# amolahinge/739-839-federated-learning-using-grpc

Measured on AMD Instinct MI355X. Metric: rounds/sec + samples/sec/client, 2-conv CNN FedAvg at 1/2/4/8 MI355X clients, higher is better.
Workload: dtype bf16; 1 GPU; model=lenet, global_batch=128, parallelism=fedavg-dp1, per_client_batch=128, local_epochs_per_round=1, eval_per_round=True, eval_split=full-per-client, data_split=strided-iid, aggregation=none (single client), hip_graph=True

## Files before the change

### csrc/bindings.cpp

```cpp
#include <pybind11/pybind11.h>
#include <pybind11/stl.h>

#include <hip/hip_runtime.h>
#include <stdint.h>
#include <cmath>
#include <vector>

#include "kernels/common.h"
#include "kernels/lenet_layout.h"
#include "runtime/lenet_engine.h"

namespace py = pybind11;

namespace fedmi {
void launch_lenet_conv_fwd(hipStream_t, const uint8_t*, int, int, const bf16*, const float*, uint32_t, const int*, int,
                           bf16*, bf16*, int, bf16*, uint8_t*, uint8_t*, lenet::Stats*);
void launch_lenet_fc_eval(hipStream_t, const bf16*, const int*, int, const bf16*, const float*, float*, long,
                          lenet::Stats*);
bool stamps_enabled();
void read_stamps(unsigned long long*, bool);
void set_ks1_diag(int);
void launch_lenet_pack(hipStream_t, const float*, bf16*);
void launch_sgd_flat(hipStream_t, float*, const float*, float*, long, float, float, float, float, int, int);
void launch_server_opt(hipStream_t, float*, float*, float*, float*, long, long, int, float, float, float, float);
void launch_drift_grad(hipStream_t, int, float*, const float*, const float*, const float*, float*, float, long);
void launch_scaffold_finish(hipStream_t, const float*, float*, float*, long, long);
void launch_scaffold_begin(hipStream_t, float*, const float*, const float*, float*, float*, long);
int dp_partials(long);
void launch_dp(hipStream_t, float*, const float*, long, double*, double*, double, float, uint64_t, uint64_t, int);
int robust_partials(long);
void launch_robust_reduce(hipStream_t, const float*, long, int, long, int, float*, long long*, long long*);
void launch_ef_delta(hipStream_t, const float*, const float*, const float*, float*, long);
size_t topk_state_bytes();
size_t topk_overflow_offset();
void launch_topk_ef(hipStream_t, const float*, const float*, float*, long, int, void*, int*, unsigned*, int*, float*);
void launch_scatter_add_ranked(hipStream_t, float*, const int*, const float*, int, long, float, long);
void launch_quant_int8(hipStream_t, const float*, long, signed char*, float*, float*);
void launch_dequant_accum(hipStream_t, const signed char*, const float*, int, long, float*, float);
}

using namespace fedmi;

void fedmi_bind_cnn(py::module_& m);
void fedmi_bind_comm(py::module_& m);
void fedmi_bind_zoo(py::module_& m);
void fedmi_bind_io(py::module_& m);

template <typename T>
static T* P(uintptr_t p) { return reinterpret_cast<T*>(p); }
static hipStream_t S(uintptr_t s) { return reinterpret_cast<hipStream_t>(s); }

static void check_last(const char* what) { check_hip(hipGetLastError(), what); }

static LeNetBuffers buffers_from(const py::dict& d) {
  auto get = [&](const char* k) -> uintptr_t { return d.contains(k) ? d[k].cast<uintptr_t>() : 0; };
  LeNetBuffers b;
  b.train_images = P<const uint8_t>(get("train_images"));
  b.train_labels = P<const int>(get("train_labels"));
  b.n_train = d.contains("n_train") ? d["n_train"].cast<int>() : 0;
  b.params = P<float>(get("params"));
  b.mom = P<float>(get("mom"));
  b.pk = P<bf16>(get("pk"));
  b.act2 = P<bf16>(get("act2"));
  b.act2_rows = d.contains("act2_rows") ? d["act2_rows"].cast<int>() : 0;
  b.act2T = P<bf16>(get("act2T"));
  b.h1 = P<bf16>(get("h1"));
  b.dact2 = P<float>(get("dact2"));
  b.dZ1T = P<bf16>(get("dZ1T"));
  b.conv_slab = P<float>(get("conv_slab"));
  b.eval_part = P<float>(get("eval_part"));
  b.eval_part_floats = d.contains("eval_part_floats") ? d["eval_part_floats"].cast<long>() : 0;
  b.train_stats = P<lenet::Stats>(get("train_stats"));
  b.eval_stats = P<lenet::Stats>(get("eval_stats"));
  b.round_ctr = P<int>(get("round_ctr"));
  return b;
}

static void fedmi_bind(py::module_& m) {
  fedmi_bind_cnn(m);
  fedmi_bind_comm(m);
  fedmi_bind_zoo(m);
  fedmi_bind_io(m);
  m.def("stamps_enabled", &stamps_enabled);
  m.def("set_ks1_diag", &set_ks1_diag);
  m.def("read_stamps", [](bool clear) {
    const size_t n = (size_t)FEDMI_STAMP_KERNELS * FEDMI_STAMP_WGS * FEDMI_STAMP_SLOTS;
    std::vector<unsigned long long> buf(n, 0ull);
    read_stamps(buf.data(), clear);
    return py::bytes(reinterpret_cast<const char*>(buf.data()), n * sizeof(unsigned long long));
  }, py::arg("clear") = true);
  m.attr("STAMP_SHAPE") = py::make_tuple(FEDMI_STAMP_KERNELS, FEDMI_STAMP_WGS, FEDMI_STAMP_SLOTS);
  m.doc() = "fedmi native runtime: fused LeNet HIP kernels, graph executor, flat-buffer and compression kernels (gfx950)";

  m.def("lenet_layout", []() {
    using namespace lenet;
    py::dict d;
    d["P_C1W"] = P_C1W; d["P_C1B"] = P_C1B; d["P_C2W"] = P_C2W; d["P_C2B"] = P_C2B;
    d["P_F1W"] = P_F1W; d["P_F1B"] = P_F1B; d["P_F2W"] = P_F2W; d["P_F2B"] = P_F2B;
    d["P_F3W"] = P_F3W; d["P_F3B"] = P_F3B; d["P_TOTAL"] = P_TOTAL;
    d["CS"] = CS; d["FS"] = FS; d["F1W_N"] = F1W_N; d["DZ1_LD"] = DZ1_LD; d["PK_TOTAL"] = PK_TOTAL; d["F0"] = F0; d["F0P"] = F0P; d["NP1"] = NP1;
    d["MAX_TRAIN_BATCH"] = MAX_TRAIN_BATCH; d["FC_SPW"] = FC_SPW;
    d["IMG_BYTES"] = IMG_BYTES; d["STATS_BYTES"] = (int)sizeof(Stats);
    return d;
  });

  py::class_<SgdConfig>(m, "SgdConfig")
      .def(py::init<>())
      .def_readwrite("lr", &SgdConfig::lr)
      .def_readwrite("momentum", &SgdConfig::momentum)
      .def_readwrite("weight_decay", &SgdConfig::weight_decay);

  py::class_<LeNetEngine>(m, "LeNetEngine")
      .def(py::init([](const py::dict& bufs, float lr, float momentum, float wd, uint32_t seed, bool augment) {
             SgdConfig c;
             c.lr = lr; c.momentum = momentum; c.weight_decay = wd;
             return new LeNetEngine(buffers_from(bufs), c, seed, augment);
           }),
           py::arg("buffers"), py::arg("lr"), py::arg("momentum"), py::arg("weight_decay"), py::arg("seed"),
           py::arg("augment"))
      .def("set_schedule", &LeNetEngine::set_schedule)
      .def("schedule_len", &LeNetEngine::schedule_len)
      .def("step", [](LeNetEngine& e, uintptr_t st, int start, int nb, bool bump, bool reset) {
             e.step(S(st), start, nb, bump, reset);
           }, py::arg("stream"), py::arg("start"), py::arg("nb"), py::arg("bump_round") = false,
           py::arg("reset_stats") = false,
           py::call_guard<py::gil_scoped_release>())
      .def("run_epoch", [](LeNetEngine& e, uintptr_t st, bool use_graph) { e.run_epoch(S(st), use_graph); },
           py::call_guard<py::gil_scoped_release>())
      .def("eval", [](LeNetEngine& e, uintptr_t st, uintptr_t images, uintptr_t labels, int n) {
             e.eval(S(st), P<const uint8_t>(images), P<const int>(labels), n);
           }, py::arg("st"), py::arg("images"), py::arg("labels"), py::arg("n"), py::call_guard<py::gil_scoped_release>())
      .def("pack", [](LeNetEngine& e, uintptr_t st) { e.pack(S(st)); }, py::call_guard<py::gil_scoped_release>())
      .def("set_sgd", [](LeNetEngine& e, float lr, float m, float wd) {
             SgdConfig c; c.lr = lr; c.momentum = m; c.weight_decay = wd; e.set_sgd(c);
           })
      .def("graph_ready", &LeNetEngine::graph_ready);

  m.def("lenet_conv_fwd", [](uintptr_t st, uintptr_t images, int base, int nb, uintptr_t pk, uintptr_t params,
                             uint32_t seed, uintptr_t round_ctr, int augment, uintptr_t act2, uintptr_t act2T,
                             int tstride, uintptr_t pool1, uintptr_t am1, uintptr_t am2, uintptr_t zero_stats) {
    launch_lenet_conv_fwd(S(st), P<const uint8_t>(images), base, nb, P<const bf16>(pk), P<const float>(params), seed,
                          P<const int>(round_ctr), augment, P<bf16>(act2), P<bf16>(act2T), tstride, P<bf16>(pool1),
                          P<uint8_t>(am1), P<uint8_t>(am2), P<lenet::Stats>(zero_stats));
    check_last("lenet_conv_fwd");
  });
  m.def("lenet_pack", [](uintptr_t st, uintptr_t params, uintptr_t pk) {
    launch_lenet_pack(S(st), P<const float>(params), P<bf16>(pk));
    check_last("lenet_pack");
  });

  m.def("sgd_flat", [](uintptr_t st, uintptr_t p, uintptr_t g, uintptr_t buf, long n, float lr, float mo, float wd,
                       float damp, bool nesterov, bool first) {
    launch_sgd_flat(S(st), P<float>(p), P<const float>(g), P<float>(buf), n, lr, mo, wd, damp, nesterov ? 1 : 0,
                    first ? 1 : 0);
    check_last("sgd_flat");
  });
  m.def("server_opt", [](uintptr_t st, uintptr_t x, uintptr_t anchor, uintptr_t mom, uintptr_t v, long n, long n_opt,
                         int kind, float lr, float beta1, float beta2, float tau) {
    if (kind < 0 || kind > 3) throw std::invalid_argument("server_opt: kind must be 0..3");
    if (n < 0 || n_opt < 0 || n_opt > n) throw std::invalid_argument("server_opt: need 0 <= n_opt <= n");
    if (n == 0) return;
    if (!x || !anchor || !mom || (kind != 0 && !v)) throw std::invalid_argument("server_opt: null buffer");
    if ((x | anchor | mom | v) % 16) throw std::invalid_argument("server_opt: buffers must be 16-byte aligned");
    launch_server_opt(S(st), P<float>(x), P<float>(anchor), P<float>(mom), P<float>(v), n, n_opt, kind, lr, beta1,
                      beta2, tau);
    check_last("server_opt");
  }, py::arg("stream"), py::arg("x"), py::arg("anchor"), py::arg("m"), py::arg("v"), py::arg("n"), py::arg("n_opt"),
     py::arg("kind"), py::arg("lr"), py::arg("beta1"), py::arg("beta2"), py::arg("tau"));

  m.def("dp_partials", [](long k) {
    if (k < 0) throw std::invalid_argument("dp_partials: need k >= 0");
    return dp_partials(k);
  });
  m.def("dp_privatize", [](uintptr_t st, uintptr_t x, uintptr_t anchor, long n, long k, uintptr_t partial,
                           uintptr_t stats, double clip, double z, int world, uint64_t key, uint64_t draw, int stages) {
    if (n < 0 || k < 0 || k > n) throw std::invalid_argument("dp_privatize: need 0 <= k <= n");
    if (!(clip > 0.0) || !std::isfinite(clip)) throw std::invalid_argument("dp_privatize: need a finite clip norm S > 0");
    if (!(z >= 0.0) || !std::isfinite(z)) throw std::invalid_argument("dp_privatize: need a finite noise multiplier z >= 0");
    if (world < 1) throw std::invalid_argument("dp_privatize: need world >= 1");
    if (stages < 1 || stages > 7) throw std::invalid_argument("dp_privatize: stages must be in 1..7");
    if (k == 0) return;
    if (!x || !anchor || !partial || !stats) throw std::invalid_argument("dp_privatize: null buffer");
    if ((x | anchor) % 16) throw std::invalid_argument("dp_privatize: x and anchor must be 16-byte aligned");
    if ((partial | stats) % 8) throw std::invalid_argument("dp_privatize: partial and stats must be 8-byte aligned");
    const float sigma = (float)(z * clip / std::sqrt((double)world));
    launch_dp(S(st), P<float>(x), P<const float>(anchor), k, P<double>(partial), P<double>(stats), clip, sigma, key,
              draw, stages);
    check_last("dp_privatize");
  }, py::arg("stream"), py::arg("x"), py::arg("anchor"), py::arg("n"), py::arg("k"), py::arg("partial"),
     py::arg("stats"), py::arg("clip"), py::arg("z"), py::arg("world"), py::arg("key"), py::arg("draw"),
     py::arg("stages") = 7);

  m.def("robust_partials", [](long n) {
    if (n < 0) throw std::invalid_argument("robust_partials: need n >= 0");
    return robust_partials(n);
  });
  m.def("robust_reduce", [](uintptr_t st, uintptr_t rows, long ld, int W, long n, int b_eff, uintptr_t out,
                            uintptr_t partial, uintptr_t stats) {
    if (W < 2 || W > 16) throw std::invalid_argument("robust_reduce: W must be in 2..16");
    if (b_eff < 0 || b_eff > (W - 1) / 2) throw std::invalid_argument("robust_reduce: need 0 <= b_eff <= (W - 1) / 2");
    if (n < 0) throw std::invalid_argument("robust_reduce: need n >= 0");
    if (ld < n || ld % 4) throw std::invalid_argument("robust_reduce: the row stride ld must be >= n and a multiple of 4");
    if (!rows || !out || !partial || !stats) throw std::invalid_argument("robust_reduce: null buffer");
    if ((rows | out) % 16) throw std::invalid_argument("robust_reduce: rows and out must be 16-byte aligned");
    if ((partial | stats) % 8) throw std::invalid_argument("robust_reduce: partial and stats must be 8-byte aligned");
    if (n == 0) return;
    launch_robust_reduce(S(st), P<const float>(rows), ld, W, n, b_eff, P<float>(out), P<long long>(partial),
                         P<long long>(stats));
    check_last("robust_reduce");
  }, py::arg("stream"), py::arg("rows"), py::arg("ld"), py::arg("W"), py::arg("n"), py::arg("b_eff"), py::arg("out"),
     py::arg("partial"), py::arg("stats"));

  m.def("drift_grad", [](uintptr_t st, int kind, uintptr_t g, uintptr_t p, uintptr_t anchor, uintptr_t corr,
                         uintptr_t acc, float mu, long n) {
    if (kind < 0 || kind > 1) throw std::invalid_argument("drift_grad: kind must be 0 (fedprox) or 1 (scaffold)");
    if (n < 0) throw std::invalid_argument("drift_grad: need n >= 0");
    if (n == 0) return;
    if (!g || (kind == 0 ? (!p || !anchor) : (!corr || !acc))) throw std::invalid_argument("drift_grad: null buffer");
    if ((g | p | anchor | corr | acc) % 16) throw std::invalid_argument("drift_grad: buffers must be 16-byte aligned");
    launch_drift_grad(S(st), kind, P<float>(g), P<const float>(p), P<const float>(anchor), P<const float>(corr),
                      P<float>(acc), mu, n);
    check_last("drift_grad");
  }, py::arg("stream"), py::arg("kind"), py::arg("g"), py::arg("p"), py::arg("anchor"), py::arg("corr"),
     py::arg("acc"), py::arg("mu"), py::arg("n"));
  m.def("scaffold_finish", [](uintptr_t st, uintptr_t acc, uintptr_t ci, uintptr_t delta, long K, long n) {
    if (K < 1) throw std::invalid_argument("scaffold_finish: need K >= 1 (no SGD step was counted this round)");
    if (n < 0) throw std::invalid_argument("scaffold_finish: need n >= 0");
    if (n == 0) return;
    if (!acc || !ci || !delta) throw std::invalid_argument("scaffold_finish: null buffer");
    if ((acc | ci | delta) % 16) throw std::invalid_argument("scaffold_finish: buffers must be 16-byte aligned");
    launch_scaffold_finish(S(st), P<const float>(acc), P<float>(ci), P<float>(delta), K, n);
    check_last("scaffold_finish");
  }, py::arg("stream"), py::arg("acc"), py::arg("ci"), py::arg("delta"), py::arg("K"), py::arg("n"));
  m.def("scaffold_begin", [](uintptr_t st, uintptr_t c, uintptr_t dmean, uintptr_t ci, uintptr_t corr, uintptr_t acc,
                             long n) {
    if (n < 0) throw std::invalid_argument("scaffold_begin: need n >= 0");
    if (n == 0) return;
    if (!c || !dmean || !ci || !corr || !acc) throw std::invalid_argument("scaffold_begin: null buffer");
    if ((c | dmean | ci | corr | acc) % 16) throw std::invalid_argument("scaffold_begin: buffers must be 16-byte aligned");
    launch_scaffold_begin(S(st), P<float>(c), P<const float>(dmean), P<const float>(ci), P<float>(corr),
                          P<float>(acc), n);
    check_last("scaffold_begin");
  }, py::arg("stream"), py::arg("c"), py::arg("dmean"), py::arg("ci"), py::arg("corr"), py::arg("acc"), py::arg("n"));

  m.def("topk_state_bytes", &topk_state_bytes);
  m.def("topk_overflow_offset", &topk_overflow_offset);
  m.def("topk_ef", [](uintptr_t st, uintptr_t x, uintptr_t g, uintptr_t residual, long n, int k, uintptr_t state,
                      uintptr_t cidx, uintptr_t ckey, uintptr_t idx, uintptr_t val) {
    if (k <= 0 || k > n) throw std::invalid_argument("topk_ef: need 0 < k <= n");
    if (n >= (1L << 30)) throw std::invalid_argument("topk_ef: n must be < 2^30 (int32 indices, 2n scratch)");
    if (!x || !g || !residual || !state || !cidx || !ckey || !idx || !val) throw std::invalid_argument("topk_ef: null buffer");
    launch_topk_ef(S(st), P<const float>(x), P<const float>(g), P<float>(residual), n, k, P<void>(state), P<int>(cidx),
                   P<unsigned>(ckey), P<int>(idx), P<float>(val));
    check_last("topk_ef");
  }, py::arg("stream"), py::arg("x"), py::arg("g"), py::arg("residual"), py::arg("n"), py::arg("k"), py::arg("state"),
     py::arg("cidx"), py::arg("ckey"), py::arg("idx"), py::arg("val"));
  m.def("ef_delta", [](uintptr_t st, uintptr_t local, uintptr_t global, uintptr_t residual, uintptr_t d, long n) {
    if (n < 0) throw std::invalid_argument("ef_delta: need n >= 0");
    if (n == 0) return;
    if (!local || !global || !d) throw std::invalid_argument("ef_delta: null buffer (only residual may be 0)");
    launch_ef_delta(S(st), P<const float>(local), P<const float>(global), P<const float>(residual), P<float>(d), n);
    check_last("ef_delta");
  });
  m.def("scatter_add_ranked", [](uintptr_t st, uintptr_t out, uintptr_t idx, uintptr_t val, int R, long m_, float scale,
                                 long n) {
    if (R <= 0) throw std::invalid_argument("scatter_add_ranked: R must be > 0");
    if (m_ < 0 || n < 0) throw std::invalid_argument("scatter_add_ranked: need m >= 0 and n >= 0");
    if (m_ == 0 || n == 0) return;
    if (!out || !idx || !val) throw std::invalid_argument("scatter_add_ranked: null buffer");
    launch_scatter_add_ranked(S(st), P<float>(out), P<const int>(idx), P<const float>(val), R, m_, scale, n);
    check_last("scatter_add_ranked");
  });
  m.def("quant_int8", [](uintptr_t st, uintptr_t d, long n, uintptr_t q, uintptr_t scales, uintptr_t residual) {
    if (n < 0) throw std::invalid_argument("quant_int8: need n >= 0");
    if (n == 0) return;
    if (!d || !q || !scales) throw std::invalid_argument("quant_int8: null buffer (only residual may be 0)");
    launch_quant_int8(S(st), P<const float>(d), n, P<signed char>(q), P<float>(scales), P<float>(residual));
    check_last("quant_int8");
  });
  m.def("dequant_accum", [](uintptr_t st, uintptr_t q, uintptr_t scales, int R, long n, uintptr_t out, float scale) {
    if (R <= 0) throw std::invalid_argument("dequant_accum: R must be > 0");
    if (n < 0) throw std::invalid_argument("dequant_accum: need n >= 0");
    if (n == 0) return;
    if (!q || !scales || !out) throw std::invalid_argument("dequant_accum: null buffer");
    launch_dequant_accum(S(st), P<const signed char>(q), P<const float>(scales), R, n, P<float>(out), scale);
    check_last("dequant_accum");
  });
}

#ifndef FEDMI_MODULE
#define FEDMI_MODULE _fedmi_native
#endif
PYBIND11_MODULE(FEDMI_MODULE, m) { fedmi_bind(m); }
```

### csrc/kernels/lenet_kernels.hip

```cpp
#include <stdexcept>

#include "common.h"
#include "lenet_layout.h"

using namespace lenet;

#ifdef FEDMI_STAMPS
__device__ unsigned long long fedmi_stamps[FEDMI_STAMP_KERNELS][FEDMI_STAMP_WGS][FEDMI_STAMP_SLOTS];
__device__ int fedmi_ks1_diag;
#endif

namespace {

constexpr int NT_FWD = 512;
constexpr int NW_FWD = NT_FWD / 64;
constexpr int NT_CONV = 1024;
constexpr int NW_CONV = NT_CONV / 64;
constexpr int NT_FC = 512;

__constant__ float kMean[3] = {0.4914f, 0.4822f, 0.4465f};
__constant__ float kInvStd[3] = {1.f / 0.2023f, 1.f / 0.1994f, 1.f / 0.2010f};

FEDMI_DEV bf16x8 ld8(const bf16* p) { return *reinterpret_cast<const bf16x8*>(p); }

FEDMI_DEV bf16x8 ld8_b64x2(const bf16* p) {
  typedef __bf16 bf16x4 __attribute__((ext_vector_type(4)));
  const bf16x4 lo = *reinterpret_cast<const bf16x4*>(p);
  const bf16x4 hi = *reinterpret_cast<const bf16x4*>(p + 4);
  bf16x8 r;
#pragma unroll
  for (int j = 0; j < 4; ++j) { r[j] = lo[j]; r[j + 4] = hi[j]; }
  return r;
}

struct Aug { int i0, j0, flip; };
FEDMI_DEV Aug aug_params(int augment, uint32_t seed, const int* round_ctr, int gidx) {
  Aug a{4, 4, 0};
  if (augment) {
    const uint32_t h = hash3(seed, (uint32_t)round_ctr[0], (uint32_t)gidx);
    a.i0 = (int)(h % 9u);
    a.j0 = (int)((h >> 8) % 9u);
    a.flip = (int)((h >> 16) & 1u);
  }
  return a;
}

FEDMI_DEV float aug_pixel(const uint8_t* raw, const Aug& a, int c, int y, int x) {
  const int sy = y + a.i0 - 4;
  const int sx = (a.flip ? 31 - x : x) + a.j0 - 4;
  float v = 0.f;
  if (sy >= 0 && sy < IMG && sx >= 0 && sx < IMG) v = (float)raw[c * 1024 + sy * 32 + sx] * (1.f / 255.f);
  return (v - kMean[c]) * kInvStd[c];
}

FEDMI_DEV void load_raw(const uint8_t* __restrict__ img, uint8_t* raw) {
  if ((int)threadIdx.x < IMG_BYTES / 16)
    reinterpret_cast<uint4*>(raw)[threadIdx.x] = reinterpret_cast<const uint4*>(img)[threadIdx.x];
}

template <int NT>
FEDMI_DEV void zero_lds(void* p, int bytes) {
  uint4* q = reinterpret_cast<uint4*>(p);
  const uint4 z = make_uint4(0, 0, 0, 0);
  for (int e = threadIdx.x; e < bytes / 16; e += NT) q[e] = z;
}

}

__global__ __launch_bounds__(NT_FWD, 6) void lenet_conv_fwd(
    const uint8_t* __restrict__ images, int sample_base, int nb,
    const bf16* __restrict__ pk, const float* __restrict__ params,
    uint32_t seed, const int* __restrict__ round_ctr, int augment,
    bf16* __restrict__ act2,
    bf16* __restrict__ act2T,
    int tstride,
    bf16* __restrict__ pool1_out,
    uint8_t* __restrict__ am1_out,
    uint8_t* __restrict__ am2_out,
    Stats* __restrict__ zero_stats)
{
  constexpr int XCL = 36 * 40 * 4, P1CL = 14 * 14 * 8;
  constexpr int O_X = 3072, O_C1 = O_X + XCL * 2, O_P1 = O_C1 + NPOS1 * 8 * 4, O_C2 = O_P1 + P1CL * 2,
                O_END = O_C2 + C2 * NPOS2 * 4;
  __shared__ __attribute__((aligned(16))) unsigned char smem[O_END];
  uint8_t* raw = smem;
  bf16* xcl = reinterpret_cast<bf16*>(smem + O_X);
  float* c1 = reinterpret_cast<float*>(smem + O_C1);
  bf16* p1cl = reinterpret_cast<bf16*>(smem + O_P1);
  float* c2 = reinterpret_cast<float*>(smem + O_C2);

  const int s = blockIdx.x;
  if (s >= nb) return;
  [[maybe_unused]] const int stamp_wg = s;
  const int gidx = sample_base + s;
  const int tid = threadIdx.x, lane = lane_id(), wave = wave_id();
  const int kq = (lane >> 4) * 8, n16 = lane & 15, rq = (lane >> 4) * 4;
  if (zero_stats != nullptr && s == 0 && tid == 0) *zero_stats = Stats{0.f, 0, 0, 0};
  FEDMI_STAMP(0, 0);

  bf16x8 wr1[4], wr2[7];
  load_raw(images + (size_t)gidx * IMG_BYTES, raw);
  zero_lds<NT_FWD>(xcl, XCL * 2);
#pragma unroll
  for (int ks = 0; ks < 4; ++ks) wr1[ks] = ld8(pk + PK_W1C + n16 * K1C + ks * 32 + kq);
#pragma unroll
  for (int ks = 0; ks < 7; ++ks) wr2[ks] = ld8(pk + PK_W2C + n16 * K2C + ks * 32 + kq);
  int go1[4], go2[7];
#pragma unroll
  for (int ks = 0; ks < 4; ++ks) {
    const int g = ks * 4 + (lane >> 4);
    go1[ks] = g < 15 ? ((g / 3) * 40 + 2 * (g % 3)) * 4 : 0;
  }
#pragma unroll
  for (int ks = 0; ks < 7; ++ks) {
    const int g = ks * 4 + (lane >> 4);
    go2[ks] = g < 25 ? ((g / 5) * P1 + (g % 5)) * 8 : 0;
  }
  const float bias1 = n16 < C1 ? params[P_C1B + n16] : 0.f;
  const float bias2 = params[P_C2B + n16];
  const Aug a = aug_params(augment, seed, round_ctr, gidx);
  __syncthreads();
  bf16x8 wb1[4];
#pragma unroll
  for (int ks = 0; ks < 4; ++ks) wb1[ks] = wr1[ks];
  for (int e = tid; e < IMG_BYTES; e += NT_FWD) {
    const int c = e >> 10, y = (e >> 5) & 31, x = e & 31;
    xcl[(y * 40 + x) * 4 + c] = (bf16)aug_pixel(raw, a, c, y, x);
  }
  __syncthreads();
  FEDMI_STAMP(0, 1);

  {
    const float bias = bias1;
    for (int t = wave; t < NPOS1 / 16; t += 2 * NW_FWD) {
      const int tb = t + NW_FWD;
      const bool two = tb < NPOS1 / 16;
      const int pa = t * 16 + n16, pb = (two ? tb : t) * 16 + n16;
      const bf16* xa = xcl + ((pa / O1) * 40 + pa % O1) * 4;
      const bf16* xbb = xcl + ((pb / O1) * 40 + pb % O1) * 4;
      bf16x8 fa[4], fb[4];
#pragma unroll
      for (int ks = 0; ks < 4; ++ks) {
        fa[ks] = ld8_b64x2(xa + go1[ks]);
        fb[ks] = ld8_b64x2(xbb + go1[ks]);
      }
      f32x4 acc = zero4(), accb = zero4();
#pragma unroll
      for (int ks = 0; ks < 4; ++ks) {
        acc = mfma16(fa[ks], wb1[ks], acc);
        accb = mfma16(fb[ks], wb1[ks], accb);
      }
      if (n16 < C1) {
#pragma unroll
        for (int r = 0; r < 4; ++r) c1[(t * 16 + rq + r) * 8 + n16] = fmaxf(acc[r] + bias, 0.f);
        if (two) {
#pragma unroll
          for (int r = 0; r < 4; ++r) c1[(tb * 16 + rq + r) * 8 + n16] = fmaxf(accb[r] + bias, 0.f);
        }
      }
    }
  }
  __syncthreads();
  FEDMI_STAMP(0, 2);

  for (int e = tid; e < P1CL; e += NT_FWD) {
    const int pos = e >> 3, c = e & 7;
    bf16 mb = (bf16)0.f;
    if (c < C1) {
      const int py = pos / P1, px = pos - py * P1;
      const float* w = c1 + ((2 * py) * O1 + 2 * px) * 8 + c;
      float m = w[0]; int am = 0;
      if (w[8] > m) { m = w[8]; am = 1; }
      if (w[O1 * 8] > m) { m = w[O1 * 8]; am = 2; }
      if (w[O1 * 8 + 8] > m) { m = w[O1 * 8 + 8]; am = 3; }
      mb = (bf16)m;
      if (pool1_out) {
        pool1_out[(size_t)s * NP1 + c * 196 + pos] = mb;
        am1_out[(size_t)s * NP1 + c * 196 + pos] = (uint8_t)am;
      }
    }
    p1cl[e] = mb;
  }
  __syncthreads();
  FEDMI_STAMP(0, 3);

  if (wave < 7) {
    const int t = wave;
    const float bias = bias2;
    int pos = t * 16 + n16;
    if (pos >= NPOS2) pos = 0;
    const int py = pos / O2, px = pos - py * O2;
    const bf16* pb = p1cl + (py * P1 + px) * 8;
    f32x4 acc = zero4();
#pragma unroll
    for (int ks = 0; ks < 7; ++ks) acc = mfma16(ld8(pb + go2[ks]), wr2[ks], acc);
#pragma unroll
    for (int r = 0; r < 4; ++r) {
      const int p = t * 16 + rq + r;
      if (p < NPOS2) c2[p * 16 + n16] = fmaxf(acc[r] + bias, 0.f);
    }
  }
  __syncthreads();
  FEDMI_STAMP(0, 4);

  for (int e = tid; e < F0P; e += NT_FWD) {
    bf16 mb = (bf16)0.f;
    if (e < F0) {
      const int o = e / 25, rem = e - o * 25, py = rem / P2, px = rem - py * P2;
      const float* w = c2 + ((2 * py) * O2 + 2 * px) * 16 + o;
      float m = w[0]; int am = 0;
      if (w[16] > m) { m = w[16]; am = 1; }
      if (w[O2 * 16] > m) { m = w[O2 * 16]; am = 2; }
      if (w[O2 * 16 + 16] > m) { m = w[O2 * 16 + 16]; am = 3; }
      mb = (bf16)m;
      if (am2_out) am2_out[(size_t)s * F0 + e] = (uint8_t)am;
    }
    act2[(size_t)s * F0P + e] = mb;
    if (act2T) act2T[(size_t)e * tstride + s] = mb;
  }
  FEDMI_STAMP(0, 5);
}

__global__ __launch_bounds__(NT_FC) void lenet_fc_eval(
    const bf16* __restrict__ act2, const int* __restrict__ labels, int nb,
    const bf16* __restrict__ pk, const float* __restrict__ params, float* __restrict__ part)
{
  constexpr int SX_LD = F0P + 8;
  constexpr int XCH = F0P / 8;
  __shared__ __attribute__((aligned(16))) bf16 sX[16 * SX_LD];
  __shared__ __attribute__((aligned(16))) bf16 sH1[16 * 128];
  __shared__ __attribute__((aligned(16))) bf16 sH2[16 * 96];
  __shared__ float sZ[16 * 16];
  const int tid = threadIdx.x, lane = lane_id(), wave = wave_id();
  const int kq = (lane >> 4) * 8, n16 = lane & 15, rq = (lane >> 4) * 4;
  const int mt = blockIdx.x, s0 = mt * FC_SPW;
  const int ns = min(FC_SPW, nb - s0);
  if (ns <= 0) return;

  const int nf1 = wave * 16 + n16;
  bf16x8 w1f[13];
#pragma unroll
  for (int ks = 0; ks < 13; ++ks) w1f[ks] = ld8(pk + PK_FC1 + nf1 * F0P + ks * 32 + kq);
  const float b1 = params[P_F1B + min(nf1, F1 - 1)];
  const int nf2 = (wave < 6 ? wave : 0) * 16 + n16;
  const float b2 = params[P_F2B + min(nf2, F2 - 1)];
  const float b3 = params[P_F3B + min(n16, NCLS - 1)];
  bf16x8 w2f[4], w3f[3];
  if (wave < 6) {
#pragma unroll
    for (int ks = 0; ks < 4; ++ks) w2f[ks] = ld8(pk + PK_FC2 + nf2 * 128 + ks * 32 + kq);
  }
  if (wave == 0) {
#pragma unroll
    for (int ks = 0; ks < 3; ++ks) w3f[ks] = ld8(pk + PK_FC3 + n16 * 96 + ks * 32 + kq);
  }
  uint4 xv[2] = {make_uint4(0, 0, 0, 0), make_uint4(0, 0, 0, 0)};
#pragma unroll
  for (int u = 0; u < 2; ++u) {
    const int e = tid + u * NT_FC;
    if (e < 16 * XCH) {
      const int r = e / XCH;
      xv[u] = reinterpret_cast<const uint4*>(act2 + (size_t)(s0 + min(r, ns - 1)) * F0P)[e - r * XCH];
      if (r >= ns) xv[u] = make_uint4(0, 0, 0, 0);
    }
  }
#pragma unroll
  for (int u = 0; u < 2; ++u) {
    const int e = tid + u * NT_FC;
    if (e < 16 * XCH) {
      const int r = e / XCH;
      *reinterpret_cast<uint4*>(sX + r * SX_LD + (e - r * XCH) * 8) = xv[u];
    }
  }
  __syncthreads();

  {
    const bf16* xa = sX + n16 * SX_LD + kq;
    f32x4 acc = zero4();
#pragma unroll
    for (int ks = 0; ks < 13; ++ks) acc = mfma16(ld8(xa + ks * 32), w1f[ks], acc);
#pragma unroll
    for (int r = 0; r < 4; ++r) {
      const int sr = rq + r;
      sH1[sr * 128 + nf1] = (bf16)((nf1 < F1 && sr < ns) ? fmaxf(acc[r] + b1, 0.f) : 0.f);
    }
  }
  __syncthreads();
  if (wave < 6) {
    const bf16* ha = sH1 + n16 * 128 + kq;
    f32x4 acc = zero4();
#pragma unroll
    for (int ks = 0; ks < 4; ++ks) acc = mfma16(ld8(ha + ks * 32), w2f[ks], acc);
#pragma unroll
    for (int r = 0; r < 4; ++r) {
      const int sr = rq + r;
      sH2[sr * 96 + nf2] = (bf16)((nf2 < F2 && sr < ns) ? fmaxf(acc[r] + b2, 0.f) : 0.f);
    }
  }
  __syncthreads();
  if (wave == 0) {
    const bf16* ha = sH2 + n16 * 96 + kq;
    f32x4 acc = zero4();
#pragma unroll
    for (int ks = 0; ks < 3; ++ks) acc = mfma16(ld8(ha + ks * 32), w3f[ks], acc);
#pragma unroll
    for (int r = 0; r < 4; ++r) sZ[(rq + r) * 16 + n16] = acc[r] + b3;
  }
  __syncthreads();
  if (wave == 0) {
    float loss = 0.f, corr = 0.f;
    if (lane < ns) {
      float z[NCLS];
#pragma unroll
      for (int n = 0; n < NCLS; ++n) z[n] = sZ[lane * 16 + n];
      float mx = z[0]; int am = 0;
#pragma unroll
      for (int n = 1; n < NCLS; ++n) if (z[n] > mx) { mx = z[n]; am = n; }
      float se = 0.f;
#pragma unroll
      for (int n = 0; n < NCLS; ++n) se += __expf(z[n] - mx);
      const int y = labels[s0 + lane];
      float zy = 0.f;
#pragma unroll
      for (int n = 0; n < NCLS; ++n) zy = (n == y) ? z[n] : zy;
      loss = mx + __logf(se) - zy;
      corr = (am == y) ? 1.f : 0.f;
    }
    loss = wave_sum(loss);
    corr = wave_sum(corr);
    if (lane == 0) {
      part[2 * mt] = loss;
      part[2 * mt + 1] = corr;
    }
  }
}

constexpr int BW_XROW = 40, BW_XS_C = 32 * BW_XROW + 72, BW_XS_S = 3 * BW_XS_C + 48;
constexpr int BW_XSH = 5 * BW_XS_S;
constexpr int BW_P1SH = 5 * 6 * 14 * 16;
constexpr int BW_DY2W = 16 * 160;
constexpr int BW_DY2S = 24;
constexpr int BW_DY2C = 18 * 18 * BW_DY2S;
constexpr int BW_DY1S = 904;
constexpr int BW_DY1 = 6 * BW_DY1S;
constexpr int BW_WDGS = KDGP + 8;
constexpr int BW_O_XSH = 0, BW_O_P1SH = BW_O_XSH + BW_XSH * 2, BW_O_DY2W = BW_O_P1SH + BW_P1SH * 2,
              BW_O_DY2C = BW_O_DY2W + BW_DY2W * 2, BW_O_DY1 = BW_O_DY2C + BW_DY2C * 2,
              BW_O_DW1 = BW_O_DY1 + BW_DY1 * 2, BW_O_DB = BW_O_DW1 + 3 * 6 * 80 * 4, BW_SCRATCH = BW_O_DB + 64 * 4;

struct BwdLds {
  const uint8_t* raw;
  const bf16* p1r;
  const uint8_t* am1s;
  const uint8_t* am2s;
  const float* dxs;
  const bf16* wdg;
  bf16* xsh; bf16* p1sh; bf16* dY2w; bf16* dY2c; bf16* dY1; float* db; float* w1part;
};

FEDMI_DEV BwdLds bwd_lds(unsigned char* scratch, const uint8_t* raw, const bf16* p1r, const uint8_t* am1s,
                         const uint8_t* am2s, const float* dxs, const bf16* wdg) {
  BwdLds L;
  L.raw = raw; L.p1r = p1r; L.am1s = am1s; L.am2s = am2s; L.dxs = dxs; L.wdg = wdg;
  L.xsh = reinterpret_cast<bf16*>(scratch + BW_O_XSH);
  L.p1sh = reinterpret_cast<bf16*>(scratch + BW_O_P1SH);
  L.dY2w = reinterpret_cast<bf16*>(scratch + BW_O_DY2W);
  L.dY2c = reinterpret_cast<bf16*>(scratch + BW_O_DY2C);
  L.dY1 = reinterpret_cast<bf16*>(scratch + BW_O_DY1);
  L.w1part = reinterpret_cast<float*>(scratch + BW_O_DW1);
  L.db = reinterpret_cast<float*>(scratch + BW_O_DB);
  return L;
}

FEDMI_DEV void bwd_zero(const BwdLds& L) {
  zero_lds<NT_CONV>(L.dY2w, BW_DY2W * 2);
  zero_lds<NT_CONV>(L.dY2c, BW_DY2C * 2);
  zero_lds<NT_CONV>(L.dY1, BW_DY1 * 2);
  const int tid = threadIdx.x;
  if (tid < 512) {
    const int sh = 1 + (tid >> 7), c = (tid >> 5) & 3, y = tid & 31;
    if (c < 3) *reinterpret_cast<uint2*>(L.xsh + sh * BW_XS_S + c * BW_XS_C + y * BW_XROW + 28) = make_uint2(0, 0);
  } else if (tid < 512 + BW_P1SH / 16) {
    *reinterpret_cast<uint4*>(L.p1sh + (tid - 512) * 16 + 8) = make_uint4(0, 0, 0, 0);
  }
  if (tid < 64) L.db[tid] = 0.f;
}
static_assert((BW_XS_S * 2) % 8 == 0 && (BW_XS_C * 2) % 8 == 0 && (BW_XROW * 2) % 8 == 0 && BW_O_P1SH % 16 == 0,
              "tail clears are aligned 8 / 16-byte stores");
static_assert(512 + BW_P1SH / 16 <= NT_CONV, "one tail clear per thread");

FEDMI_DEV void store_shifted_pairs(bf16* row, int copy_stride, int x, unsigned p01, unsigned p12) {
#pragma unroll
  for (int sh = 0; sh < 5; ++sh) {
    if (sh & 1) {
      if (x + 1 >= sh) *reinterpret_cast<unsigned*>(row + sh * copy_stride + 1 - sh) = p12;
    } else {
      if (x >= sh) *reinterpret_cast<unsigned*>(row + sh * copy_stride - sh) = p01;
    }
  }
}
FEDMI_DEV unsigned pack2(bf16 lo, bf16 hi) {
  return (unsigned)__builtin_bit_cast(unsigned short, lo) | ((unsigned)__builtin_bit_cast(unsigned short, hi) << 16);
}
FEDMI_DEV void bwd_build_shifted_img(const BwdLds& L, const bf16* xcl, int tid, int nthr) {
  for (int e = tid; e < 3 * IMG * (IMG / 2); e += nthr) {
    const int c = e >> 9, y = (e >> 4) & 31, x = 2 * (e & 15);
    const bf16* px = xcl + (y * 40 + x) * 4 + c;
    const bf16 v0 = px[0], v1 = px[4], v2 = px[8];
    store_shifted_pairs(L.xsh + c * BW_XS_C + y * BW_XROW + x, BW_XS_S, x, pack2(v0, v1), pack2(v1, v2));
  }
}
FEDMI_DEV void bwd_build_shifted_p1(const BwdLds& L, int tid, int nthr) {
  for (int e = tid; e < C1 * P1 * 8; e += nthr) {
    const int rw = e >> 3, x = 2 * (e & 7);
    if (x >= P1) continue;
    const bf16* pv = L.p1r + rw * P1 + x;
    const bf16 v0 = pv[0], v1 = pv[1], v2 = x + 2 < P1 ? pv[2] : (bf16)0.f;
    store_shifted_pairs(L.p1sh + rw * 16 + x, 6 * 14 * 16, x, pack2(v0, v1), pack2(v1, v2));
  }
}
static_assert(BW_XS_S % 2 == 0 && BW_XS_C % 2 == 0 && BW_XROW % 2 == 0 && BW_O_P1SH % 4 == 0, "pair stores are 4-byte aligned");

FEDMI_DEV void bwd_main(const BwdLds& L, float* __restrict__ slab, int sk, int stamp_wg) {
  (void)sk; (void)stamp_wg;
  int lane = lane_id();
  asm volatile("" : "+v"(lane));
  const int tid = threadIdx.x, wave = wave_id();
  const int kq = (lane >> 4) * 8, n16 = lane & 15, rq = (lane >> 4) * 4;
  float* db = L.db;
  if (tid < C2 * 32) {
    const int o = tid >> 5, rem = tid & 31;
    float g = 0.f;
    if (rem < 25) {
      const int f = o * 25 + rem, py = rem / P2, px = rem - py * P2;
      const int am = L.am2s[f];
      const int y = 2 * py + (am >> 1), x = 2 * px + (am & 1);
      g = L.dxs[f];
      const bf16 gb = (bf16)g;
      L.dY2w[o * 160 + y * 16 + x] = gb;
      L.dY2c[((y + 4) * 18 + (x + 4)) * BW_DY2S + o] = gb;
    }
#pragma unroll
    for (int w = 1; w < 32; w <<= 1) g += __shfl_xor(g, w, 64);
    if (rem == 0) db[o] = g;
  }
  __syncthreads();
  FEDMI_STAMP(sk, 2);

  for (int t = wave - 7; t >= 0 && t < 10; t += 9) {
    const int kk = t * 16 + n16;
    const int kc = kk < 150 ? kk : 0;
    const int c = kc / 25, rs = kc - c * 25, r = rs / 5, sc = rs - r * 5;
    const bf16* bb = L.p1sh + ((sc * 6 + c) * 14 + r) * 16 + (kq & 15);
    f32x4 acc = zero4();
#pragma unroll
    for (int ks = 0; ks < 5; ++ks) {
      const int i = 2 * ks + (kq >> 4);
      acc = mfma16(ld8(L.dY2w + n16 * 160 + ks * 32 + kq), ld8(bb + i * 16), acc);
    }
    if (kk < 150) {
#pragma unroll
      for (int rr = 0; rr < 4; ++rr) slab[P_C2W + (rq + rr) * 150 + kk] = acc[rr];
    }
  }

  if (wave < 7) {
    int koff[13];
#pragma unroll
    for (int ks = 0; ks < 13; ++ks) {
      const int G = ks * 4 + (lane >> 4), g = G >> 1;
      const int r = g / 5, sc = g - r * 5;
      koff[ks] = g < 25 ? (-r * 18 - sc) * BW_DY2S + (G & 1) * 8 : 0;
    }
    const int ta = 2 * wave, tb = 2 * wave + 1;
    int pa = ta * 16 + n16, pb = tb * 16 + n16;
    if (pa >= 196) pa = 0;
    if (pb >= 196) pb = 0;
    const bf16* ga = L.dY2c + (((pa / P1) + 4) * 18 + (pa % P1 + 4)) * BW_DY2S;
    const bf16* gbb = L.dY2c + (((pb / P1) + 4) * 18 + (pb % P1 + 4)) * BW_DY2S;
    const bf16* wb = L.wdg + min(n16, C1) * BW_WDGS + kq;
    f32x4 acc[2] = {zero4(), zero4()};
#pragma unroll
    for (int ks = 0; ks < 13; ++ks) {
      const bf16x8 w = ld8(wb + ks * 32);
      acc[0] = mfma16(ld8(ga + koff[ks]), w, acc[0]);
      acc[1] = mfma16(ld8(gbb + koff[ks]), w, acc[1]);
    }
    FEDMI_STAMP(sk, 6);
    float csum = 0.f;
    if (n16 < C1) {
      const int c = n16;
#pragma unroll
      for (int h = 0; h < 2; ++h) {
        const int t = h ? tb : ta;
        const int p0 = t * 16 + rq;
        if (p0 < 196) {
          const int py0 = p0 / P1, px0 = p0 - py0 * P1;
          const uint2 pv = *reinterpret_cast<const uint2*>(L.p1r + c * 196 + p0);
          const unsigned av = *reinterpret_cast<const unsigned*>(L.am1s + c * 196 + p0);
#pragma unroll
          for (int rr = 0; rr < 4; ++rr) {
            const int wrap = px0 + rr >= P1, py = py0 + wrap, px = px0 + rr - wrap * P1;
            const unsigned w = rr < 2 ? pv.x : pv.y;
            const float pooled = __builtin_bit_cast(float, (rr & 1) ? (w & 0xffff0000u) : (w << 16));
            const float g = pooled > 0.f ? acc[h][rr] : 0.f;
            const int am = (av >> (8 * rr)) & 3;
            const int yy = 2 * py + (am >> 1), xx = 2 * px + (am & 1);
            L.dY1[c * BW_DY1S + yy * 32 + xx] = (bf16)g;
            csum += g;
          }
        }
      }
    }
    csum += __shfl_xor(csum, 16, 64);
    csum += __shfl_xor(csum, 32, 64);
    if (n16 < C1 && lane < 16) db[16 + wave * C1 + n16] = csum;
    FEDMI_STAMP(sk, 7);
  }
  __syncthreads();
  FEDMI_STAMP(sk, 3);

  if (wave < 15) {
    const int nt = wave % 5, part = wave / 5;
    const int ks0 = part * 10, ks1 = min(ks0 + 10, O1);
    const int kk = nt * 16 + n16;
    const int kc = kk < 75 ? kk : kk - 64;
    const int c = kc / 25, rs = kc - c * 25, r = rs / 5, sc = rs - r * 5;
    const bf16* bb = L.xsh + sc * BW_XS_S + c * BW_XS_C + r * BW_XROW + kq;
    const bf16* ab = L.dY1 + min(n16, C1 - 1) * BW_DY1S + kq;
    const bool arow = n16 < C1;
    f32x4 acc0 = zero4(), acc1 = zero4();
    int ks = ks0;
    for (; ks + 1 < ks1; ks += 2) {
      bf16x8 a0 = ld8(ab + ks * 32), a1 = ld8(ab + ks * 32 + 32);
      if (!arow) { a0 = zero8(); a1 = zero8(); }
      acc0 = mfma16(a0, ld8(bb + ks * BW_XROW), acc0);
      acc1 = mfma16(a1, ld8(bb + (ks + 1) * BW_XROW), acc1);
    }
    if (ks < ks1) {
      bf16x8 a0 = ld8(ab + ks * 32);
      if (!arow) a0 = zero8();
      acc0 = mfma16(a0, ld8(bb + ks * BW_XROW), acc0);
    }
#pragma unroll
    for (int rr = 0; rr < 4; ++rr) {
      const int o = rq + rr;
      if (o < C1 && kk < 75) L.w1part[(part * 6 + o) * 80 + kk] = acc0[rr] + acc1[rr];
    }
  }
  __syncthreads();
  FEDMI_STAMP(sk, 4);
  if (tid < C1 * 128) {
    const int o = tid >> 7, kk = tid & 127;
    if (kk < 75)
      slab[P_C1W + o * 75 + kk] = L.w1part[o * 80 + kk] + L.w1part[(6 + o) * 80 + kk] + L.w1part[(12 + o) * 80 + kk];
  }
  if (tid < C1) {
    float b = 0.f;
#pragma unroll
    for (int w = 0; w < 7; ++w) b += db[16 + w * C1 + tid];
    slab[P_C1B + tid] = b;
  }
  if (tid < C2) slab[P_C2B + tid] = db[tid];
  FEDMI_STAMP(sk, 5);
}

constexpr int AUX_H2T = 0;
constexpr int AUX_DZ2T = AUX_H2T + 96 * 128 * 2;
constexpr int AUX_DZ3T = AUX_DZ2T + 96 * 128 * 2;
constexpr int FCB_N = 224;
constexpr int AUX_FCB = AUX_DZ3T + 16 * 128 * 2;
constexpr int AUX_LOSS = AUX_FCB + MAX_TRAIN_BATCH * FCB_N * 4;
constexpr int AUX_CORR = AUX_LOSS + MAX_TRAIN_BATCH * 4;
constexpr int AUX_BYTES = AUX_CORR + MAX_TRAIN_BATCH * 4;
static_assert(AUX_BYTES <= MAX_TRAIN_BATCH * F0 * 4, "FC side buffers must fit in dact2");

constexpr int S_O_RAW = 0, S_O_P1R = 3072, S_O_AM1 = S_O_P1R + 2368, S_O_AM2 = S_O_AM1 + 1184,
              S_O_X = S_O_AM2 + 416, S_O_DX = S_O_X + F0P * 2, S_O_WDG = S_O_DX + F0 * 4,
              S_O_FC = S_O_WDG + 16 * BW_WDGS * 2, S_O_W1C = S_O_FC + 2048, S_O_W2C = S_O_W1C + 16 * 136 * 2,
              S_O_SCR = S_O_W2C + 16 * 232 * 2;
constexpr int S_W1C_LD = 136, S_W2C_LD = 232;
constexpr int S_O_RED = S_O_SCR + BW_SCRATCH;
constexpr int S_R_XCL = 128 * 4 * 4, S_R_P1 = S_R_XCL + 36 * 40 * 4 * 2, S_R_END = S_R_P1 + 14 * 14 * 8 * 2;
static_assert(S_R_END <= NW_CONV * F0P * 4 && S_O_RED % 16 == 0, "forward images fit behind the fc1 partials");
constexpr int S_O_W3 = S_O_RED + NW_CONV * F0P * 4;
constexpr int S_END = S_O_W3 + 16 * 96 * 2;
static_assert(S_END <= 160 * 1024, "KS1 LDS");
static_assert(S_O_P1R % 8 == 0 && S_O_AM1 % 4 == 0, "pool1 backward reads 4 positions per access");
constexpr int SF_H1 = 0, SF_H2 = 128, SF_Z = 224, SF_DZ3 = 240, SF_DZ2 = 256, SF_DZ1 = 352, SF_END = 480;
static_assert(SF_END * 4 <= 2048, "FC scratch");

FEDMI_DEV float dot8(const bf16x8& a, const bf16x8& b, float acc) {
#pragma unroll
  for (int j = 0; j < 8; ++j) acc += (float)a[j] * (float)b[j];
  return acc;
}
FEDMI_DEV float dot8f(const float* a, const bf16x8& b, float acc) {
#pragma unroll
  for (int j = 0; j < 8; ++j) acc += a[j] * (float)b[j];
  return acc;
}
FEDMI_DEV float sum8lanes(float v) {
  v += __shfl_xor(v, 1, 64);
  v += __shfl_xor(v, 2, 64);
  v += __shfl_xor(v, 4, 64);
  return v;
}
FEDMI_DEV float bfr(float v) { return (float)(bf16)v; }
FEDMI_DEV float row_sum16(float v) {
  v += __builtin_bit_cast(float, __builtin_amdgcn_mov_dpp(__builtin_bit_cast(int, v), 0x128, 0xf, 0xf, false));
  v += __builtin_bit_cast(float, __builtin_amdgcn_mov_dpp(__builtin_bit_cast(int, v), 0x124, 0xf, 0xf, false));
  v += __builtin_bit_cast(float, __builtin_amdgcn_mov_dpp(__builtin_bit_cast(int, v), 0x122, 0xf, 0xf, false));
  v += __builtin_bit_cast(float, __builtin_amdgcn_mov_dpp(__builtin_bit_cast(int, v), 0x121, 0xf, 0xf, false));
  return v;
}

__global__ __launch_bounds__(NT_CONV) void lenet_sample_step(
    const uint8_t* __restrict__ images, int sample_base, int nb,
    const bf16* __restrict__ pk, const float* __restrict__ params,
    uint32_t seed, const int* __restrict__ round_ctr, int augment,
    const int* __restrict__ labels,
    bf16* __restrict__ act2T,
    bf16* __restrict__ h1T,
    unsigned char* __restrict__ aux,
    bf16* __restrict__ dZ1T,
    float* __restrict__ conv_slab)
{
  __shared__ __attribute__((aligned(16))) unsigned char smem[S_END];
  const int s = blockIdx.x;
  if (s >= nb) return;
  [[maybe_unused]] const int stamp_wg = s;
  const int gidx = sample_base + s;
  const int tid = threadIdx.x, lane = lane_id(), wave = wave_id();
  const int kq = (lane >> 4) * 8, n16 = lane & 15, rq = (lane >> 4) * 4;
  uint8_t* raw = smem + S_O_RAW;
  bf16* p1r = reinterpret_cast<bf16*>(smem + S_O_P1R);
  uint8_t* am1s = smem + S_O_AM1;
  uint8_t* am2s = smem + S_O_AM2;
  bf16* xrow = reinterpret_cast<bf16*>(smem + S_O_X);
  float* dxs = reinterpret_cast<float*>(smem + S_O_DX);
  bf16* wdg = reinterpret_cast<bf16*>(smem + S_O_WDG);
  float* fcs = reinterpret_cast<float*>(smem + S_O_FC);
  float* red = reinterpret_cast<float*>(smem + S_O_RED);
  bf16* xcl = reinterpret_cast<bf16*>(smem + S_O_RED + S_R_XCL);
  bf16* p1cl = reinterpret_cast<bf16*>(smem + S_O_RED + S_R_P1);
  const BwdLds L = bwd_lds(smem + S_O_SCR, raw, p1r, am1s, am2s, dxs, wdg);
  FEDMI_STAMP(0, 0);

  bf16* w1c = reinterpret_cast<bf16*>(smem + S_O_W1C);
  bf16* w2c = reinterpret_cast<bf16*>(smem + S_O_W2C);
  bf16* w3s = reinterpret_cast<bf16*>(smem + S_O_W3);
  float bias1, bias2;
  Aug a;
  {
    constexpr int NI = IMG_BYTES / 16, NWD = 16 * KDGP / 8, NW1 = 16 * K1C / 8, NW2 = 16 * K2C / 8, NW3 = 16 * 96 / 8;
    constexpr int E1 = NI, E2 = E1 + NWD, E3 = E2 + NW1, E4 = E3 + NW2, E5 = E4 + NW3;
    static_assert(E5 <= 2 * NT_CONV, "stage: two chunks per thread");
    uint4 v[2] = {make_uint4(0, 0, 0, 0), make_uint4(0, 0, 0, 0)};
#ifdef FEDMI_STAMPS
    const int dg = fedmi_ks1_diag;
    const size_t img_sample = (dg & 2) ? 0 : (size_t)gidx;
    const int lim = (dg & 1) ? E1 : E5;
#else
    const size_t img_sample = (size_t)gidx;
    constexpr int lim = E5;
#endif
#pragma unroll
    for (int u = 0; u < 2; ++u) {
      const int e = tid + u * NT_CONV;
      if (e < E1) v[u] = reinterpret_cast<const uint4*>(images + img_sample * IMG_BYTES)[e];
      else if (e >= lim) {}
      else if (e < E2) v[u] = reinterpret_cast<const uint4*>(pk + PK_W2DG)[e - E1];
      else if (e < E3) v[u] = reinterpret_cast<const uint4*>(pk + PK_W1C)[e - E2];
      else if (e < E4) v[u] = reinterpret_cast<const uint4*>(pk + PK_W2C)[e - E3];
      else if (e < E5) v[u] = reinterpret_cast<const uint4*>(pk + PK_FC3)[e - E4];
    }
    bias1 = n16 < C1 ? params[P_C1B + n16] : 0.f;
    bias2 = params[P_C2B + n16];
    a = aug_params(augment, seed, round_ctr, gidx);
    zero_lds<NT_CONV>(xcl, 36 * 40 * 4 * 2);
    bwd_zero(L);
#pragma unroll
    for (int u = 0; u < 2; ++u) {
      const int e = tid + u * NT_CONV;
      if (e < E1) {
        reinterpret_cast<uint4*>(raw)[e] = v[u];
      } else if (e < E2) {
        const int w = e - E1, row = w / (KDGP / 8), col = w - row * (KDGP / 8);
        reinterpret_cast<uint4*>(wdg + row * BW_WDGS)[col] = v[u];
      } else if (e < E3) {
        const int w = e - E2, row = w / (K1C / 8), col = w - row * (K1C / 8);
        reinterpret_cast<uint4*>(w1c + row * S_W1C_LD)[col] = v[u];
      } else if (e < E4) {
        const int w = e - E3, row = w / (K2C / 8), col = w - row * (K2C / 8);
        reinterpret_cast<uint4*>(w2c + row * S_W2C_LD)[col] = v[u];
      } else if (e < E5) {
        reinterpret_cast<uint4*>(w3s)[e - E4] = v[u];
      }
    }
  }
  int go1[4];
#pragma unroll
  for (int ks = 0; ks < 4; ++ks) {
    const int g = ks * 4 + (lane >> 4);
    go1[ks] = g < 15 ? ((g / 3) * 40 + 2 * (g % 3)) * 4 : 0;
  }
  __syncthreads();
  FEDMI_STAMP(1, 7);
  bf16x8 wb1[4];
#pragma unroll
  for (int ks = 0; ks < 4; ++ks) wb1[ks] = ld8(w1c + n16 * S_W1C_LD + ks * 32 + kq);
  for (int e = tid; e < IMG_BYTES; e += NT_CONV) {
    const int c = e >> 10, y = (e >> 5) & 31, x = e & 31;
    xcl[(y * 40 + x) * 4 + c] = (bf16)aug_pixel(raw, a, c, y, x);
  }
  __syncthreads();
  FEDMI_STAMP(0, 1);

  auto c1_row = [&](int tt) {
    const int q = tt * 4 + (n16 >> 2), y = 2 * (q / P1) + ((n16 >> 1) & 1), x = 2 * (q % P1) + (n16 & 1);
    return xcl + (y * 40 + x) * 4;
  };
  auto pool1 = [&](const f32x4& v, int tt) {
    if (n16 < 8) {
      const int q = tt * 4 + (lane >> 4);
      float m = fmaxf(v[0] + bias1, 0.f), c;
      int am = 0;
      c = fmaxf(v[1] + bias1, 0.f); if (c > m) { m = c; am = 1; }
      c = fmaxf(v[2] + bias1, 0.f); if (c > m) { m = c; am = 2; }
      c = fmaxf(v[3] + bias1, 0.f); if (c > m) { m = c; am = 3; }
      const bf16 mb = (bf16)m;
      p1cl[q * 8 + n16] = mb;
      if (n16 < C1) {
        p1r[n16 * 196 + q] = mb;
        am1s[n16 * 196 + q] = (uint8_t)am;
      }
    }
  };
  for (int t = wave; t < NPOS1 / 16; t += 2 * NW_CONV) {
    const int tb = t + NW_CONV;
    const bool two = tb < NPOS1 / 16;
    const bf16* xa = c1_row(t);
    const bf16* xbb = c1_row(two ? tb : t);
    bf16x8 fa[4], fb[4];
#pragma unroll
    for (int ks = 0; ks < 4; ++ks) {
      fa[ks] = ld8_b64x2(xa + go1[ks]);
      fb[ks] = ld8_b64x2(xbb + go1[ks]);
    }
    f32x4 acc = zero4(), accb = zero4();
#pragma unroll
    for (int ks = 0; ks < 4; ++ks) {
      acc = mfma16(fa[ks], wb1[ks], acc);
      accb = mfma16(fb[ks], wb1[ks], accb);
    }
    pool1(acc, t);
    if (two) pool1(accb, tb);
  }
  const int fn = tid >> 3, fq = tid & 7;
  constexpr int KCH = F0P / 8;
  const int kc = min(lane, KCH - 1);
  bf16x8 w1r[8];
#pragma unroll
  for (int m = 0; m < 8; ++m) w1r[m] = ld8(pk + PK_FC1 + (wave + 16 * m) * F0P + kc * 8);
  __syncthreads();
  FEDMI_STAMP(0, 2);
  FEDMI_STAMP(0, 3);

  if (wave < 7) {
    const int t = wave;
    int q = t * 4 + (n16 >> 2);
    if (q >= P2 * P2) q = 0;
    const int y = 2 * (q / P2) + ((n16 >> 1) & 1), x = 2 * (q % P2) + (n16 & 1);
    const bf16* pb = p1cl + (y * P1 + x) * 8;
    const bf16* wb = w2c + n16 * S_W2C_LD + kq;
    int go2[7];
#pragma unroll
    for (int ks = 0; ks < 7; ++ks) {
      const int g = ks * 4 + (lane >> 4);
      go2[ks] = g < 25 ? ((g / 5) * P1 + (g % 5)) * 8 : 0;
    }
    f32x4 acc = zero4();
#pragma unroll
    for (int ks = 0; ks < 7; ++ks) acc = mfma16(ld8(pb + go2[ks]), ld8(wb + ks * 32), acc);
    const int qo = t * 4 + (lane >> 4);
    if (qo < P2 * P2) {
      float m = fmaxf(acc[0] + bias2, 0.f), c;
      int am = 0;
      c = fmaxf(acc[1] + bias2, 0.f); if (c > m) { m = c; am = 1; }
      c = fmaxf(acc[2] + bias2, 0.f); if (c > m) { m = c; am = 2; }
      c = fmaxf(acc[3] + bias2, 0.f); if (c > m) { m = c; am = 3; }
      const bf16 mb = (bf16)m;
      const int e = n16 * (P2 * P2) + qo;
      am2s[e] = (uint8_t)am;
      xrow[e] = mb;
      act2T[(size_t)e * MAX_TRAIN_BATCH + s] = mb;
    }
    bwd_build_shifted_p1(L, tid, 7 * 64);
  } else {
    if (tid < 7 * 64 + (F0P - F0)) {
      const int e = F0 + tid - 7 * 64;
      xrow[e] = (bf16)0.f;
      act2T[(size_t)e * MAX_TRAIN_BATCH + s] = (bf16)0.f;
    }
    bwd_build_shifted_img(L, xcl, tid - 7 * 64, NT_CONV - 7 * 64);
  }
  FEDMI_STAMP(0, 4);
  const int n2 = fn < 96 ? fn : 95;
  bf16x8 w2v[2];
#pragma unroll
  for (int i = 0; i < 2; ++i) w2v[i] = ld8(pk + PK_FC2 + n2 * 128 + fq * 8 + 64 * i);
  const int label = labels[s];
  const float fb1 = params[P_F1B + min(tid & 127, F1 - 1)];
  const float fb2 = params[P_F2B + min(fn, F2 - 1)];
  const float fb3 = params[P_F3B + min(fn, NCLS - 1)];
  __syncthreads();
  FEDMI_STAMP(0, 5);

  unsigned char* auxp = aux;
  float* fcb = reinterpret_cast<float*>(auxp + AUX_FCB) + (size_t)s * FCB_N;
  {
    const bf16x8 xv = ld8(xrow + kc * 8);
#pragma unroll
    for (int m = 0; m < 8; ++m) {
      const float p = row_sum16(lane < KCH ? dot8(xv, w1r[m], 0.f) : 0.f);
      if ((lane & 15) == 0) red[(wave + 16 * m) * 4 + (lane >> 4)] = p;
    }
  }
  bf16x8 w2t[2];
#pragma unroll
  for (int i = 0; i < 2; ++i) w2t[i] = ld8(pk + PK_FC2T + fn * 96 + min(fq * 8 + 64 * i, 88));
  __syncthreads();
  if (tid < 128) {
    const float* r = red + tid * 4;
    const float h = bfr(tid < F1 ? fmaxf(((r[0] + r[1]) + r[2]) + r[3] + fb1, 0.f) : 0.f);
    fcs[SF_H1 + tid] = h;
    h1T[(size_t)tid * MAX_TRAIN_BATCH + s] = (bf16)h;
  }
  __syncthreads();

  FEDMI_STAMP(1, 0);
  if (fn < 96) {
    float acc = 0.f;
#pragma unroll
    for (int i = 0; i < 2; ++i) acc = dot8f(fcs + SF_H1 + fq * 8 + 64 * i, w2v[i], acc);
    acc = sum8lanes(acc);
    if (fq == 0) {
      const float h = bfr(fn < F2 ? fmaxf(acc + fb2, 0.f) : 0.f);
      fcs[SF_H2 + fn] = h;
      reinterpret_cast<bf16*>(auxp + AUX_H2T)[(size_t)fn * MAX_TRAIN_BATCH + s] = (bf16)h;
    }
  }
  __syncthreads();
  FEDMI_STAMP(1, 1);
  if (fn < 16) {
    float acc = 0.f;
#pragma unroll
    for (int i = 0; i < 2; ++i)
      if (fq * 8 + 64 * i < 96) acc = dot8f(fcs + SF_H2 + fq * 8 + 64 * i, ld8(w3s + fn * 96 + fq * 8 + 64 * i), acc);
    acc = sum8lanes(acc);
    if (fq == 0) fcs[SF_Z + fn] = fn < NCLS ? acc + fb3 : 0.f;
  }
  __syncthreads();
  FEDMI_STAMP(1, 2);
  if (wave == 0) {
    int ln = lane;
    asm volatile("" : "+v"(ln));
    const int n = ln & 15;
    const float zn = n < NCLS ? fcs[SF_Z + n] : -INFINITY;
    float mx = zn;
#pragma unroll
    for (int o = 1; o < 16; o <<= 1) mx = fmaxf(mx, __shfl_xor(mx, o, 64));
    float cand = (zn == mx) ? (float)n : 16.f;
#pragma unroll
    for (int o = 1; o < 16; o <<= 1) cand = fminf(cand, __shfl_xor(cand, o, 64));
    float se = n < NCLS ? __expf(zn - mx) : 0.f;
#pragma unroll
    for (int o = 1; o < 16; o <<= 1) se += __shfl_xor(se, o, 64);
    const float lse = mx + __logf(se);
    const int y = label;
    const float zy = __shfl(zn, y, 64);
    const float d = n < NCLS ? (__expf(zn - lse) - (n == y ? 1.f : 0.f)) * (1.f / (float)nb) : 0.f;
    if (lane < 16) {
      fcs[SF_DZ3 + n] = bfr(d);
      reinterpret_cast<bf16*>(auxp + AUX_DZ3T)[(size_t)n * MAX_TRAIN_BATCH + s] = (bf16)d;
      if (n < NCLS) fcb[204 + n] = d;
    }
    if (lane == 0) {
      reinterpret_cast<float*>(auxp + AUX_LOSS)[s] = lse - zy;
      reinterpret_cast<float*>(auxp + AUX_CORR)[s] = ((int)cand == y) ? 1.f : 0.f;
    }
  }
  __syncthreads();
  FEDMI_STAMP(1, 3);
  if (tid < 96) {
    float acc = 0.f;
#pragma unroll
    for (int n = 0; n < NCLS; ++n) acc += fcs[SF_DZ3 + n] * (float)w3s[n * 96 + tid];
    const float g = (tid < F2 && fcs[SF_H2 + tid] > 0.f) ? acc : 0.f;
    fcs[SF_DZ2 + tid] = bfr(g);
    reinterpret_cast<bf16*>(auxp + AUX_DZ2T)[(size_t)tid * MAX_TRAIN_BATCH + s] = (bf16)g;
    if (tid < F2) fcb[120 + tid] = g;
  }
  __syncthreads();
  FEDMI_STAMP(1, 4);
  {
    float acc = 0.f;
#pragma unroll
    for (int i = 0; i < 2; ++i)
      if (fq * 8 + 64 * i < 96) acc = dot8f(fcs + SF_DZ2 + fq * 8 + 64 * i, w2t[i], acc);
    acc = sum8lanes(acc);
    if (fq == 0) {
      const float g = (fn < F1 && fcs[SF_H1 + fn] > 0.f) ? acc : 0.f;
      fcs[SF_DZ1 + fn] = bfr(g);
      dZ1T[(size_t)fn * DZ1_LD + s] = (bf16)g;
      if (fn < F1) fcb[fn] = g;
    }
  }
  __syncthreads();
  FEDMI_STAMP(1, 5);
  {
    float d[8];
#pragma unroll
    for (int j = 0; j < 8; ++j) d[j] = 0.f;
#pragma unroll
    for (int m = 0; m < 8; ++m) {
      const float g = fcs[SF_DZ1 + wave + 16 * m];
#pragma unroll
      for (int j = 0; j < 8; ++j) d[j] += g * (float)w1r[m][j];
    }
    if (lane < KCH) {
      float4* o = reinterpret_cast<float4*>(red + wave * F0P + lane * 8);
      o[0] = make_float4(d[0], d[1], d[2], d[3]);
      o[1] = make_float4(d[4], d[5], d[6], d[7]);
    }
  }
  __syncthreads();
  if (tid < F0) {
    float acc = 0.f;
#pragma unroll
    for (int w = 0; w < NW_CONV; ++w) acc += red[w * F0P + tid];
    dxs[tid] = (float)xrow[tid] > 0.f ? acc : 0.f;
  }
  __syncthreads();
  FEDMI_STAMP(0, 6);
  bwd_main(L, conv_slab + (size_t)s * CS, 2, stamp_wg);
}

FEDMI_DEV void pack_one(int i, float w, bf16* __restrict__ pk) {
  const bf16 v = (bf16)w;
  if (i < P_C1B) {
    const int o = i / 75, k = i - o * 75, c = k / 25, rs = k - c * 25, r = rs / 5, s = rs - r * 5;
    pk[PK_W1C + o * K1C + (r * 3 + (s >> 1)) * 8 + (s & 1) * 4 + c] = v;
  } else if (i < P_C2W) {
  } else if (i < P_C2B) {
    const int j = i - P_C2W, o = j / 150, k = j - o * 150, c = k / 25, rs = k - c * 25;
    pk[PK_W2C + o * K2C + rs * 8 + c] = v;
    pk[PK_W2DG + c * KDGP + rs * 16 + o] = v;
  } else if (i < P_F1W) {
  } else if (i < P_F1B) {
    const int j = i - P_F1W, n = j / F0, f = j - n * F0;
    pk[PK_FC1 + n * F0P + f] = v;
  } else if (i < P_F2W) {
  } else if (i < P_F2B) {
    const int j = i - P_F2W, n = j / F1, f = j - n * F1;
    pk[PK_FC2 + n * 128 + f] = v;
    pk[PK_FC2T + f * 96 + n] = v;
  } else if (i < P_F3W) {
  } else if (i < P_F3B) {
    const int j = i - P_F3W, n = j / F2, f = j - n * F2;
    pk[PK_FC3 + n * 96 + f] = v;
  }
}

__global__ __launch_bounds__(256) void lenet_pack(const float* __restrict__ params, bf16* __restrict__ pk) {
  const int i = blockIdx.x * 256 + threadIdx.x;
  if (i < P_TOTAL) pack_one(i, params[i], pk);
}

constexpr int SGD_NA = (CS + 15) / 16;

FEDMI_DEV void sgd_apply(int i, float grad, float p, float m, float* __restrict__ params, float* __restrict__ mom,
                         bf16* __restrict__ pk, float lr, float momentum, float wd) {
  const float d = grad + wd * p;
  const float b = momentum * m + d;
  const float np = p - lr * b;
  mom[i] = b;
  params[i] = np;
  pack_one(i, np, pk);
}

FEDMI_DEV bf16x8 mask_cols(bf16x8 v, int s0, int nb) {
  if (s0 + 8 <= nb) return v;
#pragma unroll
  for (int j = 0; j < 8; ++j)
    if (s0 + j >= nb) v[j] = (bf16)0.f;
  return v;
}

FEDMI_DEV f32x4 batch_tile(const bf16* __restrict__ a, const bf16* __restrict__ b, int nb,
                           const float* __restrict__ params, const float* __restrict__ mom, const int* idx,
                           float* p, float* m) {
  const int lane = lane_id(), kq = (lane >> 4) * 8, n16 = lane & 15;
  bf16x8 av[4], bv[4];
#pragma unroll
  for (int ks = 0; ks < 4; ++ks) {
    av[ks] = ld8(a + n16 * MAX_TRAIN_BATCH + ks * 32 + kq);
    bv[ks] = ld8(b + n16 * MAX_TRAIN_BATCH + ks * 32 + kq);
  }
#pragma unroll
  for (int r = 0; r < 4; ++r) {
    p[r] = params[idx[r] >= 0 ? idx[r] : 0];
    m[r] = mom[idx[r] >= 0 ? idx[r] : 0];
  }
  f32x4 acc = zero4();
  if (nb == MAX_TRAIN_BATCH) {
#pragma unroll
    for (int ks = 0; ks < 4; ++ks) acc = mfma16(av[ks], bv[ks], acc);
  } else {
#pragma unroll
    for (int ks = 0; ks < 4; ++ks)
      acc = mfma16(mask_cols(av[ks], ks * 32 + kq, nb), mask_cols(bv[ks], ks * 32 + kq, nb), acc);
  }
  return acc;
}

constexpr int SGD2_NB = (8 * 25 + 3) / 4;
constexpr int SGD2_NC = (6 * 8 + 3) / 4;
constexpr int SGD2_ND = (6 + 3) / 4;
constexpr int SGD2_NE = 4;
constexpr int SGD2_GRID = SGD_NA + SGD2_NB + SGD2_NC + SGD2_ND + SGD2_NE + 1;

__global__ __launch_bounds__(256) void lenet_sgd2(
    float* __restrict__ params, float* __restrict__ mom, bf16* __restrict__ pk,
    const float* __restrict__ conv_slab, int nb,
    const bf16* __restrict__ act2T, const bf16* __restrict__ h1T, const unsigned char* __restrict__ aux,
    const bf16* __restrict__ dZ1T, float lr, float momentum, float wd,
    int* __restrict__ round_ctr, Stats* __restrict__ stats)
{
  __shared__ float red[16][17];
  const int b = blockIdx.x, tid = threadIdx.x, wave = wave_id(), lane = lane_id();
  const int n16 = lane & 15, rq = (lane >> 4) * 4;
  [[maybe_unused]] const int stamp_wg = b;
  FEDMI_STAMP(3, 0);
  if (b < SGD_NA) {
    const int pl = tid & 15, g = tid >> 4;
    const int i = b * 16 + pl;
    float p = 0.f, m = 0.f;
    if (g == 0 && i < CS) { p = params[i]; m = mom[i]; }
    float sum = 0.f;
    if (i < CS) {
      float v[MAX_TRAIN_BATCH / 16];
#pragma unroll
      for (int u = 0; u < MAX_TRAIN_BATCH / 16; ++u) v[u] = conv_slab[(size_t)min(g + 16 * u, nb - 1) * CS + i];
#pragma unroll
      for (int u = 0; u < MAX_TRAIN_BATCH / 16; ++u) sum += g + 16 * u < nb ? v[u] : 0.f;
    }
    red[g][pl] = sum;
    __syncthreads();
    if (g == 0 && i < CS) {
      float tot = 0.f;
#pragma unroll
      for (int q = 0; q < 16; ++q) tot += red[q][pl];
      sgd_apply(i, tot, p, m, params, mom, pk, lr, momentum, wd);
    }
  } else if (b < SGD_NA + SGD2_NB) {
    const int t = (b - SGD_NA) * 4 + wave;
    if (t < 200) {
      const int nt = t / 25, ft = t - nt * 25;
      int idx[4];
      float p[4], m[4];
#pragma unroll
      for (int r = 0; r < 4; ++r) {
        const int n = nt * 16 + rq + r, f = ft * 16 + n16;
        idx[r] = n < F1 ? P_F1W + n * F0 + f : -1;
      }
      const f32x4 acc = batch_tile(dZ1T + (size_t)nt * 16 * DZ1_LD, act2T + (size_t)ft * 16 * MAX_TRAIN_BATCH, nb,
                                   params, mom, idx, p, m);
      FEDMI_STAMP(3, 2);
#pragma unroll
      for (int r = 0; r < 4; ++r)
        if (idx[r] >= 0) sgd_apply(idx[r], acc[r], p[r], m[r], params, mom, pk, lr, momentum, wd);
      FEDMI_STAMP(3, 3);
    }
  } else if (b < SGD_NA + SGD2_NB + SGD2_NC) {
    const int t = (b - SGD_NA - SGD2_NB) * 4 + wave;
    if (t < 48) {
      const int nt = t >> 3, ft = t & 7;
      const bf16* dz2t = reinterpret_cast<const bf16*>(aux + AUX_DZ2T);
      int idx[4];
      float p[4], m[4];
#pragma unroll
      for (int r = 0; r < 4; ++r) {
        const int n = nt * 16 + rq + r, f = ft * 16 + n16;
        idx[r] = (n < F2 && f < F1) ? P_F2W + n * F1 + f : -1;
      }
      const f32x4 acc = batch_tile(dz2t + (size_t)nt * 16 * MAX_TRAIN_BATCH, h1T + (size_t)ft * 16 * MAX_TRAIN_BATCH, nb,
                                   params, mom, idx, p, m);
#pragma unroll
      for (int r = 0; r < 4; ++r)
        if (idx[r] >= 0) sgd_apply(idx[r], acc[r], p[r], m[r], params, mom, pk, lr, momentum, wd);
    }
  } else if (b < SGD_NA + SGD2_NB + SGD2_NC + SGD2_ND) {
    const int t = (b - SGD_NA - SGD2_NB - SGD2_NC) * 4 + wave;
    if (t < 6) {
      const bf16* dz3t = reinterpret_cast<const bf16*>(aux + AUX_DZ3T);
      const bf16* h2t = reinterpret_cast<const bf16*>(aux + AUX_H2T);
      int idx[4];
      float p[4], m[4];
#pragma unroll
      for (int r = 0; r < 4; ++r) {
        const int n = rq + r, f = t * 16 + n16;
        idx[r] = (n < NCLS && f < F2) ? P_F3W + n * F2 + f : -1;
      }
      const f32x4 acc = batch_tile(dz3t, h2t + (size_t)t * 16 * MAX_TRAIN_BATCH, nb, params, mom, idx, p, m);
#pragma unroll
      for (int r = 0; r < 4; ++r)
        if (idx[r] >= 0) sgd_apply(idx[r], acc[r], p[r], m[r], params, mom, pk, lr, momentum, wd);
    }
  } else {
    const int e = b - (SGD_NA + SGD2_NB + SGD2_NC + SGD2_ND);
    const float* fcb = reinterpret_cast<const float*>(aux + AUX_FCB);
    const int j = e * 64 + (tid & 63), g = tid >> 6;
    __shared__ float bsum[4][64];
    float bp = 0.f, bm = 0.f;
    const int bi = j < 120 ? P_F1B + j : (j < 204 ? P_F2B + j - 120 : P_F3B + j - 204);
    if (e < SGD2_NE && g == 0 && j < 214) { bp = params[bi]; bm = mom[bi]; }
    if (e < SGD2_NE && j < 214) {
      float v[32];
#pragma unroll
      for (int u = 0; u < 32; ++u) v[u] = fcb[(size_t)min(g * 32 + u, nb - 1) * FCB_N + j];
      float sum = 0.f;
#pragma unroll
      for (int u = 0; u < 32; ++u) sum += g * 32 + u < nb ? v[u] : 0.f;
      bsum[g][tid & 63] = sum;
    } else if (e == SGD2_NE && g == 0 && stats != nullptr) {
      const float* lv = reinterpret_cast<const float*>(aux + AUX_LOSS);
      const float* cv = reinterpret_cast<const float*>(aux + AUX_CORR);
      float ls = 0.f, cs = 0.f;
#pragma unroll
      for (int u = 0; u < 2; ++u) {
        const int sm = lane + 64 * u;
        if (sm < nb) { ls += lv[sm]; cs += cv[sm]; }
      }
      ls = wave_sum(ls);
      cs = wave_sum(cs);
      if (lane == 0) {
        stats->loss_sum += ls;
        stats->correct += (int)(cs + 0.5f);
        stats->count += nb;
      }
    }
    __syncthreads();
    if (e < SGD2_NE && g == 0 && j < 214) {
      const float sum = (bsum[0][tid] + bsum[1][tid]) + (bsum[2][tid] + bsum[3][tid]);
      sgd_apply(bi, sum, bp, bm, params, mom, pk, lr, momentum, wd);
    }
  }
  if (b == 0 && tid == 0 && round_ctr) atomicAdd(round_ctr, 1);
  FEDMI_STAMP(3, 1);
}

namespace fedmi {

void launch_lenet_conv_fwd(hipStream_t st, const uint8_t* images, int sample_base, int nb,
                           const bf16* pk, const float* params, uint32_t seed, const int* round_ctr,
                           int augment, bf16* act2, bf16* act2T, int tstride, bf16* pool1,
                           uint8_t* am1, uint8_t* am2, Stats* zero_stats) {
  if (nb <= 0) return;
  hipLaunchKernelGGL(lenet_conv_fwd, dim3(nb), dim3(NT_FWD), 0, st, images, sample_base, nb, pk, params,
                     seed, round_ctr, augment, act2, act2T, tstride, pool1, am1, am2, zero_stats);
}

__global__ __launch_bounds__(256) void lenet_eval_stats(const float* __restrict__ part, int groups, int n,
                                                        Stats* __restrict__ stats) {
  __shared__ float rl[256], rc[256];
  float l = 0.f, c = 0.f;
  for (int g = threadIdx.x; g < groups; g += 256) { l += part[2 * g]; c += part[2 * g + 1]; }
  rl[threadIdx.x] = l;
  rc[threadIdx.x] = c;
  __syncthreads();
  for (int w = 128; w > 0; w >>= 1) {
    if (threadIdx.x < w) { rl[threadIdx.x] += rl[threadIdx.x + w]; rc[threadIdx.x] += rc[threadIdx.x + w]; }
    __syncthreads();
  }
  if (threadIdx.x == 0) {
    stats->loss_sum += rl[0];
    stats->correct += (int)(rc[0] + 0.5f);
    stats->count += n;
  }
}

void launch_lenet_fc_eval(hipStream_t st, const bf16* act2, const int* labels, int n, const bf16* pk,
                          const float* params, float* part, long part_floats, Stats* stats) {
  if (n <= 0) return;
  const int mtiles = (n + FC_SPW - 1) / FC_SPW;
  if (2L * mtiles > part_floats) throw std::invalid_argument("lenet eval: partials scratch too small");
  hipLaunchKernelGGL(lenet_fc_eval, dim3(mtiles), dim3(NT_FC), 0, st, act2, labels, n, pk, params, part);
  hipLaunchKernelGGL(lenet_eval_stats, dim3(1), dim3(256), 0, st, part, mtiles, n, stats);
}

bool stamps_enabled() {
#ifdef FEDMI_STAMPS
  return true;
#else
  return false;
#endif
}

void set_ks1_diag(int v) {
#ifdef FEDMI_STAMPS
  (void)hipMemcpyToSymbol(HIP_SYMBOL(fedmi_ks1_diag), &v, sizeof(v), 0, hipMemcpyHostToDevice);
#else
  (void)v;
#endif
}

void read_stamps(unsigned long long* host, bool clear) {
#ifdef FEDMI_STAMPS
  (void)hipMemcpyFromSymbol(host, HIP_SYMBOL(fedmi_stamps), sizeof(fedmi_stamps), 0, hipMemcpyDeviceToHost);
  if (clear) {
    static unsigned long long zeros[FEDMI_STAMP_KERNELS][FEDMI_STAMP_WGS][FEDMI_STAMP_SLOTS];
    (void)hipMemcpyToSymbol(HIP_SYMBOL(fedmi_stamps), zeros, sizeof(zeros), 0, hipMemcpyHostToDevice);
  }
#else
  (void)host;
  (void)clear;
#endif
}

__global__ void lenet_zero_stats(Stats* __restrict__ s) {
  if (threadIdx.x == 0) *s = Stats{0.f, 0, 0, 0};
}

void launch_lenet_zero_stats(hipStream_t st, Stats* s) {
  hipLaunchKernelGGL(lenet_zero_stats, dim3(1), dim3(64), 0, st, s);
}

void launch_lenet_pack(hipStream_t st, const float* params, bf16* pk) {
  hipLaunchKernelGGL(lenet_pack, dim3((P_TOTAL + 255) / 256), dim3(256), 0, st, params, pk);
}

void launch_lenet_sample_step(hipStream_t st, const uint8_t* images, int sample_base, int nb, const bf16* pk,
                              const float* params, uint32_t seed, const int* round_ctr, int augment,
                              const int* labels, bf16* act2T, bf16* h1T, float* aux, bf16* dZ1T, float* conv_slab) {
  if (nb <= 0 || nb > MAX_TRAIN_BATCH) throw std::invalid_argument("lenet_sample_step: batch must be in [1, 128]");
  hipLaunchKernelGGL(lenet_sample_step, dim3(nb), dim3(NT_CONV), 0, st, images, sample_base, nb, pk, params, seed,
                     round_ctr, augment, labels, act2T, h1T, reinterpret_cast<unsigned char*>(aux), dZ1T, conv_slab);
}

void launch_lenet_sgd2(hipStream_t st, float* params, float* mom, bf16* pk, const float* conv_slab, int nb,
                       const bf16* act2T, const bf16* h1T, const float* aux, const bf16* dZ1T, float lr,
                       float momentum, float wd, int* round_ctr, Stats* stats) {
  if (nb <= 0 || nb > MAX_TRAIN_BATCH) throw std::invalid_argument("lenet_sgd2: batch must be in [1, 128]");
  hipLaunchKernelGGL(lenet_sgd2, dim3(SGD2_GRID), dim3(256), 0, st, params, mom, pk, conv_slab, nb, act2T, h1T,
                     reinterpret_cast<const unsigned char*>(aux), dZ1T, lr, momentum, wd, round_ctr, stats);
}

}
```

### csrc/kernels/lenet_layout.h

```cpp
#pragma once

namespace lenet {

constexpr int IMG = 32, CIN = 3, C1 = 6, C2 = 16;
constexpr int O1 = 28, P1 = 14;
constexpr int O2 = 10, P2 = 5;
constexpr int NPOS1 = O1 * O1;
constexpr int NP1 = C1 * P1 * P1;
constexpr int NPOS2 = O2 * O2;
constexpr int F0 = C2 * P2 * P2;
constexpr int F0P = 416;
constexpr int F1 = 120, F2 = 84, NCLS = 10;
constexpr int IMG_BYTES = CIN * IMG * IMG;

constexpr int K1C = 128, K2C = 224, KDG = 400, KDGP = 416;

constexpr int P_C1W = 0;
constexpr int P_C1B = 450;
constexpr int P_C2W = 456;
constexpr int P_C2B = 2856;
constexpr int P_F1W = 2872;
constexpr int P_F1B = 50872;
constexpr int P_F2W = 50992;
constexpr int P_F2B = 61072;
constexpr int P_F3W = 61156;
constexpr int P_F3B = 61996;
constexpr int P_TOTAL = 62006;

constexpr int CS = P_F1W;
constexpr int FS = P_TOTAL - P_F1B;
constexpr int F1W_N = P_F1B - P_F1W;

constexpr int PK_W1C  = 0;
constexpr int PK_W2C  = PK_W1C + 16 * K1C;
constexpr int PK_W2DG = PK_W2C + 16 * K2C;
constexpr int PK_FC1  = PK_W2DG + 16 * KDGP;
constexpr int PK_FC2  = PK_FC1 + 128 * F0P;
constexpr int PK_FC2T = PK_FC2 + 96 * 128;
constexpr int PK_FC3  = PK_FC2T + 128 * 96;
constexpr int PK_TOTAL = PK_FC3 + 16 * 96;

constexpr int MAX_TRAIN_BATCH = 128;
constexpr int FC_SPW = 16;
constexpr int DZ1_LD = 128;

struct Stats {
  float loss_sum;
  int correct;
  int count;
  int pad;
};

}
```

### csrc/runtime/lenet_engine.cpp

```cpp
#include "lenet_engine.h"

#include <stdexcept>
#include <string>

namespace fedmi {

using lenet::Stats;

void launch_lenet_conv_fwd(hipStream_t, const uint8_t*, int, int, const bf16*, const float*, uint32_t,
                           const int*, int, bf16*, bf16*, int, bf16*, uint8_t*, uint8_t*, lenet::Stats*);
void launch_lenet_fc_eval(hipStream_t, const bf16*, const int*, int, const bf16*, const float*, float*, long,
                          lenet::Stats*);
void launch_lenet_pack(hipStream_t, const float*, bf16*);
void launch_lenet_zero_stats(hipStream_t, lenet::Stats*);
void launch_lenet_sample_step(hipStream_t, const uint8_t*, int, int, const bf16*, const float*, uint32_t, const int*,
                              int, const int*, bf16*, bf16*, float*, bf16*, float*);
void launch_lenet_sgd2(hipStream_t, float*, float*, bf16*, const float*, int, const bf16*, const bf16*, const float*,
                       const bf16*, float, float, float, int*, lenet::Stats*);

void check_hip(hipError_t e, const char* what) {
  if (e != hipSuccess) throw std::runtime_error(std::string("fedmi HIP error in ") + what + ": " + hipGetErrorString(e));
}

LeNetEngine::LeNetEngine(const LeNetBuffers& b, SgdConfig sgd, uint32_t seed, bool augment)
    : b_(b), sgd_(sgd), seed_(seed), augment_(augment) {
  if (!b.params || !b.mom || !b.pk || !b.act2 || !b.act2T || !b.h1 || !b.dact2 || !b.dZ1T || !b.conv_slab ||
      !b.eval_part || !b.train_stats || !b.eval_stats || !b.round_ctr)
    throw std::invalid_argument("LeNetEngine: missing device buffer");
  if (b.act2_rows < lenet::MAX_TRAIN_BATCH) throw std::invalid_argument("LeNetEngine: act2_rows < 128");
  check_hip(hipStreamCreateWithFlags(&cap_stream_, hipStreamNonBlocking), "hipStreamCreate");
}

LeNetEngine::~LeNetEngine() {
  drop_graph();
  if (cap_stream_) (void)hipStreamDestroy(cap_stream_);
}

void LeNetEngine::drop_graph() {
  if (exec_) (void)hipGraphExecDestroy(exec_);
  if (graph_) (void)hipGraphDestroy(graph_);
  exec_ = nullptr;
  graph_ = nullptr;
}

void LeNetEngine::set_schedule(const std::vector<int>& starts, const std::vector<int>& sizes) {
  if (starts.size() != sizes.size()) throw std::invalid_argument("schedule: length mismatch");
  for (size_t i = 0; i < starts.size(); ++i) {
    if (sizes[i] <= 0 || sizes[i] > lenet::MAX_TRAIN_BATCH) throw std::invalid_argument("schedule: bad batch size");
    if (starts[i] < 0 || starts[i] + sizes[i] > b_.n_train) throw std::invalid_argument("schedule: batch out of range");
  }
  starts_ = starts;
  sizes_ = sizes;
  drop_graph();
}

void LeNetEngine::set_sgd(SgdConfig sgd) {
  sgd_ = sgd;
  drop_graph();
}

void LeNetEngine::step(hipStream_t st, int start, int nb, bool bump_round, bool reset_stats) {
  using namespace lenet;
  if (nb <= 0 || nb > MAX_TRAIN_BATCH || start < 0 || start + nb > b_.n_train)
    throw std::invalid_argument("LeNetEngine::step: batch out of range");
  const int aug = augment_ ? 1 : 0;
  if (reset_stats) launch_lenet_zero_stats(st, b_.train_stats);
  launch_lenet_sample_step(st, b_.train_images, start, nb, b_.pk, b_.params, seed_, b_.round_ctr, aug,
                           b_.train_labels + start, b_.act2T, b_.h1, b_.dact2, b_.dZ1T, b_.conv_slab);
  launch_lenet_sgd2(st, b_.params, b_.mom, b_.pk, b_.conv_slab, nb, b_.act2T, b_.h1, b_.dact2, b_.dZ1T, sgd_.lr,
                    sgd_.momentum, sgd_.weight_decay, bump_round ? b_.round_ctr : nullptr, b_.train_stats);
  check_hip(hipGetLastError(), "LeNetEngine::step launch");
}

void LeNetEngine::enqueue_epoch(hipStream_t st) {
  const size_t n = starts_.size();
  for (size_t i = 0; i < n; ++i) step(st, starts_[i], sizes_[i], i + 1 == n, i == 0);
}

void LeNetEngine::run_epoch(hipStream_t st, bool use_graph) {
  if (starts_.empty()) {
    check_hip(hipMemsetAsync(b_.train_stats, 0, sizeof(Stats), st), "memset stats");
    return;
  }
  if (!use_graph) {
    enqueue_epoch(st);
    return;
  }
  if (!exec_) {
    check_hip(hipStreamBeginCapture(cap_stream_, hipStreamCaptureModeThreadLocal), "BeginCapture");
    try {
      enqueue_epoch(cap_stream_);
    } catch (...) {
      hipGraph_t g = nullptr;
      (void)hipStreamEndCapture(cap_stream_, &g);
      if (g) (void)hipGraphDestroy(g);
      throw;
    }
    check_hip(hipStreamEndCapture(cap_stream_, &graph_), "EndCapture");
    check_hip(hipGraphInstantiate(&exec_, graph_, nullptr, nullptr, 0), "GraphInstantiate");
  }
  check_hip(hipGraphLaunch(exec_, st), "GraphLaunch");
}

void LeNetEngine::eval(hipStream_t st, const uint8_t* images, const int* labels, int n) {
  using namespace lenet;
  if (n <= 0 || n > b_.act2_rows) throw std::invalid_argument("LeNetEngine::eval: n exceeds act2 capacity");
  launch_lenet_conv_fwd(st, images, 0, n, b_.pk, b_.params, seed_, b_.round_ctr, 0, b_.act2, nullptr, 0,
                        nullptr, nullptr, nullptr, b_.eval_stats);
  launch_lenet_fc_eval(st, b_.act2, labels, n, b_.pk, b_.params, b_.eval_part, b_.eval_part_floats, b_.eval_stats);
  check_hip(hipGetLastError(), "LeNetEngine::eval launch");
}

void LeNetEngine::pack(hipStream_t st) {
  launch_lenet_pack(st, b_.params, b_.pk);
  check_hip(hipGetLastError(), "LeNetEngine::pack launch");
}

}
```

### csrc/runtime/lenet_engine.h

```cpp
#pragma once
#include <hip/hip_runtime.h>
#include <stdint.h>
#include <vector>
#include "../kernels/lenet_layout.h"

namespace fedmi {

typedef __bf16 bf16;

struct LeNetBuffers {
  const uint8_t* train_images = nullptr;
  const int* train_labels = nullptr;
  int n_train = 0;
  float* params = nullptr;
  float* mom = nullptr;
  bf16* pk = nullptr;
  bf16* act2 = nullptr;
  int act2_rows = 0;
  bf16* act2T = nullptr;
  bf16* h1 = nullptr;
  float* dact2 = nullptr;
  bf16* dZ1T = nullptr;
  float* conv_slab = nullptr;
  float* eval_part = nullptr;
  long eval_part_floats = 0;
  lenet::Stats* train_stats = nullptr;
  lenet::Stats* eval_stats = nullptr;
  int* round_ctr = nullptr;
};

struct SgdConfig {
  float lr = 0.1f, momentum = 0.9f, weight_decay = 5e-4f;
};

class LeNetEngine {
 public:
  LeNetEngine(const LeNetBuffers& b, SgdConfig sgd, uint32_t seed, bool augment);
  ~LeNetEngine();
  LeNetEngine(const LeNetEngine&) = delete;
  LeNetEngine& operator=(const LeNetEngine&) = delete;

  void set_schedule(const std::vector<int>& starts, const std::vector<int>& sizes);
  int schedule_len() const { return (int)starts_.size(); }

  void step(hipStream_t st, int start, int nb, bool bump_round, bool reset_stats = false);
  void run_epoch(hipStream_t st, bool use_graph);
  void eval(hipStream_t st, const uint8_t* images, const int* labels, int n);
  void pack(hipStream_t st);
  void set_sgd(SgdConfig sgd);
  bool graph_ready() const { return exec_ != nullptr; }

 private:
  void enqueue_epoch(hipStream_t st);
  void drop_graph();

  LeNetBuffers b_;
  SgdConfig sgd_;
  uint32_t seed_;
  bool augment_;
  std::vector<int> starts_, sizes_;
  hipStream_t cap_stream_ = nullptr;
  hipGraph_t graph_ = nullptr;
  hipGraphExec_t exec_ = nullptr;
};

void check_hip(hipError_t e, const char* what);

}
```

### fedmi/engine/lenet_native.py

```python
from __future__ import annotations

from collections import OrderedDict
from typing import List, Optional

import dataclasses

import torch

from .. import native
from ..models.small import LeNet
from .base import EpochStats, LocalTrainer, TrainerConfig, ordered_views
from .data import FedDataset, ImageSet

LENET_SPEC = [
    ("conv1.weight", (6, 3, 5, 5)), ("conv1.bias", (6,)),
    ("conv2.weight", (16, 6, 5, 5)), ("conv2.bias", (16,)),
    ("fc1.weight", (120, 400)), ("fc1.bias", (120,)),
    ("fc2.weight", (84, 120)), ("fc2.bias", (84,)),
    ("fc3.weight", (10, 84)), ("fc3.bias", (10,)),
]


def _ptr(t: Optional[torch.Tensor]) -> int:
    return 0 if t is None else int(t.data_ptr())


class LeNetNativeTrainer(LocalTrainer):
    model_name = "lenet"

    def __init__(self, data: FedDataset, device: torch.device, cfg: TrainerConfig = TrainerConfig(),
                 init_state=None):
        if device.type != "cuda":
            raise ValueError("LeNetNativeTrainer runs on a GPU (use TorchTrainer on CPU)")
        if tuple(data.train.x.shape[1:]) != (3, 32, 32):
            raise ValueError("LeNet native engine expects 3x32x32 uint8 images")
        nat = native.require()
        self._nat = nat
        self.L = L = nat.lenet_layout()
        self.cfg = dataclasses.replace(cfg)
        self._device = device
        self.round_idx = 0
        with torch.cuda.device(device):
            self.train_set = data.train.to(device)
            self.test_set = data.test.to(device)
            if self.train_set.y.dtype != torch.int32:
                self.train_set.y = self.train_set.y.to(torch.int32)
            if self.test_set.y.dtype != torch.int32:
                self.test_set.y = self.test_set.y.to(torch.int32)
            z = lambda *s, dt=torch.float32: torch.zeros(*s, dtype=dt, device=device)
            B = L["MAX_TRAIN_BATCH"]
            self.params = z(L["P_TOTAL"])
            self.mom = z(L["P_TOTAL"])
            self.pk = z(L["PK_TOTAL"], dt=torch.bfloat16)
            self.act2_rows = max(B, len(self.test_set))
            self.act2 = z(self.act2_rows, L["F0P"], dt=torch.bfloat16)
            self.act2T = z(L["F0P"], B, dt=torch.bfloat16)
            self.h1 = z(B, 128, dt=torch.bfloat16)
            self.dact2 = z(B, L["F0"])
            self.dZ1T = z(L["DZ1_LD"], B, dt=torch.bfloat16)
            self.conv_slab = z(B, L["CS"])
            self.eval_part = z(2 * ((self.act2_rows + L["FC_SPW"] - 1) // L["FC_SPW"]))
            self.stats = z(2, 4, dt=torch.int32)
            self.round_ctr = z(4, dt=torch.int32)
        self._bufs = dict(
            train_images=_ptr(self.train_set.x), train_labels=_ptr(self.train_set.y), n_train=len(self.train_set),
            params=_ptr(self.params), mom=_ptr(self.mom), pk=_ptr(self.pk), act2=_ptr(self.act2),
            act2_rows=self.act2_rows, act2T=_ptr(self.act2T), h1=_ptr(self.h1), dact2=_ptr(self.dact2),
            dZ1T=_ptr(self.dZ1T), conv_slab=_ptr(self.conv_slab), eval_part=_ptr(self.eval_part),
            eval_part_floats=self.eval_part.numel(), train_stats=_ptr(self.stats[0]),
            eval_stats=_ptr(self.stats[1]), round_ctr=_ptr(self.round_ctr))
        self.engine = nat.LeNetEngine(self._bufs, cfg.lr, cfg.momentum, cfg.weight_decay, cfg.seed & 0xFFFFFFFF,
                                      bool(data.augment and cfg.augment))
        self._views = ordered_views(self.params, LENET_SPEC)
        if init_state is None:
            torch.manual_seed(cfg.seed)
            init_state = LeNet().state_dict()
        self.load_state_dict(init_state)
        self._starts: List[int] = []
        self._sizes: List[int] = []

    @property
    def device(self) -> torch.device:
        return self._device

    def _stream(self) -> int:
        return native.stream_handle(self._device)

    def state_dict(self):
        return OrderedDict(self._views)

    def load_state_dict(self, sd) -> None:
        for name, _ in LENET_SPEC:
            src = sd[name]
            self._views[name].copy_(src.to(self._device, torch.float32).view(self._views[name].shape))
        self.after_aggregate()

    def float_state(self) -> torch.Tensor:
        return self.params

    def after_aggregate(self) -> None:
        self.engine.pack(self._stream())

    def momentum_state(self) -> torch.Tensor:
        return self.mom

    def set_schedule(self, starts, sizes) -> None:
        starts, sizes = list(map(int, starts)), list(map(int, sizes))
        if (starts, sizes) != (self._starts, self._sizes):
            self.engine.set_schedule(starts, sizes)
            self._starts, self._sizes = starts, sizes

    def set_train_data(self, data: ImageSet) -> None:
        self.train_set = data.to(self._device)
        if self.train_set.y.dtype != torch.int32:
            self.train_set.y = self.train_set.y.to(torch.int32)
        self._bufs.update(train_images=_ptr(self.train_set.x), train_labels=_ptr(self.train_set.y),
                          n_train=len(self.train_set))
        self.engine = self._nat.LeNetEngine(self._bufs, self.cfg.lr, self.cfg.momentum, self.cfg.weight_decay,
                                            self.cfg.seed & 0xFFFFFFFF, bool(self.cfg.augment))
        self._starts, self._sizes = [], []

    def train_epoch(self) -> None:
        self.engine.run_epoch(self._stream(), bool(self.cfg.use_graph))
        if self._starts:
            self.round_idx += 1

    def train_step(self, start: int, nb: int, bump_round: bool = False) -> None:
        self.engine.step(self._stream(), int(start), int(nb), bool(bump_round))

    def _read_stats(self, i: int) -> EpochStats:
        return self.decode_stats(self.stats[i].cpu())

    def decode_stats(self, raw: torch.Tensor) -> EpochStats:
        raw = raw.contiguous()
        return EpochStats(float(raw[0:1].view(torch.float32).item()), int(raw[1]), int(raw[2]))

    def eval_stats_raw(self) -> torch.Tensor:
        return self.stats[1]

    def train_stats(self) -> EpochStats:
        return self._read_stats(0)

    def evaluate(self) -> None:
        self.engine.eval(self._stream(), _ptr(self.test_set.x), _ptr(self.test_set.y), len(self.test_set))

    def eval_stats(self) -> EpochStats:
        return self._read_stats(1)

    def reset_momentum(self) -> None:
        self.mom.zero_()

    def set_lr(self, lr: float) -> None:
        self.cfg.lr = float(lr)
        self.engine.set_sgd(self.cfg.lr, self.cfg.momentum, self.cfg.weight_decay)
```

Before: 5.667 million samples/s.

## Prepare next batch's augmented images inside SGD kernel, staging into xprep buffer

```diff
diff --git a/csrc/bindings.cpp b/csrc/bindings.cpp
--- a/csrc/bindings.cpp
+++ b/csrc/bindings.cpp
@@ -21,6 +21,7 @@
 void read_stamps(unsigned long long*, bool);
 void set_ks1_diag(int);
 void launch_lenet_pack(hipStream_t, const float*, bf16*);
+void launch_lenet_prep_batch(hipStream_t, const uint8_t*, int, int, uint32_t, const int*, int, bf16*);
 void launch_sgd_flat(hipStream_t, float*, const float*, float*, long, float, float, float, float, int, int);
 void launch_server_opt(hipStream_t, float*, float*, float*, float*, long, long, int, float, float, float, float);
 void launch_drift_grad(hipStream_t, int, float*, const float*, const float*, const float*, float*, float, long);
@@ -73,6 +74,7 @@
   b.train_stats = P<lenet::Stats>(get("train_stats"));
   b.eval_stats = P<lenet::Stats>(get("eval_stats"));
   b.round_ctr = P<int>(get("round_ctr"));
+  b.xprep = P<bf16>(get("xprep"));
   return b;
 }
 
@@ -101,6 +103,9 @@
     d["CS"] = CS; d["FS"] = FS; d["F1W_N"] = F1W_N; d["DZ1_LD"] = DZ1_LD; d["PK_TOTAL"] = PK_TOTAL; d["F0"] = F0; d["F0P"] = F0P; d["NP1"] = NP1;
     d["MAX_TRAIN_BATCH"] = MAX_TRAIN_BATCH; d["FC_SPW"] = FC_SPW;
     d["IMG_BYTES"] = IMG_BYTES; d["STATS_BYTES"] = (int)sizeof(Stats);
+    d["PK_W1C"] = PK_W1C; d["PK_W2C"] = PK_W2C; d["PK_W2DG"] = PK_W2DG; d["PK_FC1"] = PK_FC1;
+    d["PK_FC2"] = PK_FC2; d["PK_FC2T"] = PK_FC2T; d["PK_FC3"] = PK_FC3;
+    d["XP_H"] = XP_H; d["XP_W"] = XP_W; d["XP_C"] = XP_C; d["XP_ELEMS"] = XP_ELEMS;
     return d;
   });
 
@@ -144,6 +149,12 @@
                           P<uint8_t>(am1), P<uint8_t>(am2), P<lenet::Stats>(zero_stats));
     check_last("lenet_conv_fwd");
   });
+  m.def("lenet_prep_batch", [](uintptr_t st, uintptr_t images, int base, int nb, uint32_t seed, uintptr_t round_ctr,
+                               int augment, uintptr_t xprep) {
+    launch_lenet_prep_batch(S(st), P<const uint8_t>(images), base, nb, seed, P<const int>(round_ctr), augment,
+                            P<bf16>(xprep));
+    check_last("lenet_prep_batch");
+  });
   m.def("lenet_pack", [](uintptr_t st, uintptr_t params, uintptr_t pk) {
     launch_lenet_pack(S(st), P<const float>(params), P<bf16>(pk));
     check_last("lenet_pack");
diff --git a/csrc/kernels/lenet_kernels.hip b/csrc/kernels/lenet_kernels.hip
--- a/csrc/kernels/lenet_kernels.hip
+++ b/csrc/kernels/lenet_kernels.hip
@@ -46,6 +46,7 @@
 }
 
 FEDMI_DEV float aug_pixel(const uint8_t* raw, const Aug& a, int c, int y, int x) {
+#pragma clang fp contract(off)
   const int sy = y + a.i0 - 4;
   const int sx = (a.flip ? 31 - x : x) + a.j0 - 4;
   float v = 0.f;
@@ -56,6 +57,33 @@
 FEDMI_DEV void load_raw(const uint8_t* __restrict__ img, uint8_t* raw) {
   if ((int)threadIdx.x < IMG_BYTES / 16)
     reinterpret_cast<uint4*>(raw)[threadIdx.x] = reinterpret_cast<const uint4*>(img)[threadIdx.x];
+}
+
+constexpr int PREP_NT = 256;
+constexpr int XP_CHUNKS = XP_ELEMS / 8;
+constexpr int PREP_SPLIT = (XP_CHUNKS + PREP_NT - 1) / PREP_NT;
+FEDMI_DEV void prep_sample(const uint8_t* __restrict__ images, int gidx, int part, uint32_t seed,
+                           const int* __restrict__ round_ctr, int augment, bf16* __restrict__ xp, uint8_t* raw) {
+  const int tid = threadIdx.x;
+  uint4 v = make_uint4(0, 0, 0, 0);
+  if (tid < IMG_BYTES / 16) v = reinterpret_cast<const uint4*>(images + (size_t)gidx * IMG_BYTES)[tid];
+  const Aug a = aug_params(augment, seed, round_ctr, gidx);
+  if (tid < IMG_BYTES / 16) reinterpret_cast<uint4*>(raw)[tid] = v;
+  __syncthreads();
+  const int e = part * PREP_NT + tid;
+  if (e < XP_CHUNKS) {
+    const int y = e / (XP_W / 2), x = (e - y * (XP_W / 2)) * 2;
+    bf16x8 o;
+#pragma unroll
+    for (int j = 0; j < 8; ++j) o[j] = (bf16)0.f;
+    if (y < IMG && x < IMG) {
+#pragma unroll
+      for (int j = 0; j < 2; ++j)
+#pragma unroll
+        for (int c = 0; c < CIN; ++c) o[j * XP_C + c] = (bf16)aug_pixel(raw, a, c, y, x + j);
+    }
+    *reinterpret_cast<bf16x8*>(xp + e * 8) = o;
+  }
 }
 
 template <int NT>
@@ -349,7 +377,6 @@
               BW_O_DW1 = BW_O_DY1 + BW_DY1 * 2, BW_O_DB = BW_O_DW1 + 3 * 6 * 80 * 4, BW_SCRATCH = BW_O_DB + 64 * 4;
 
 struct BwdLds {
-  const uint8_t* raw;
   const bf16* p1r;
   const uint8_t* am1s;
   const uint8_t* am2s;
@@ -358,10 +385,10 @@
   bf16* xsh; bf16* p1sh; bf16* dY2w; bf16* dY2c; bf16* dY1; float* db; float* w1part;
 };
 
-FEDMI_DEV BwdLds bwd_lds(unsigned char* scratch, const uint8_t* raw, const bf16* p1r, const uint8_t* am1s,
+FEDMI_DEV BwdLds bwd_lds(unsigned char* scratch, const bf16* p1r, const uint8_t* am1s,
                          const uint8_t* am2s, const float* dxs, const bf16* wdg) {
   BwdLds L;
-  L.raw = raw; L.p1r = p1r; L.am1s = am1s; L.am2s = am2s; L.dxs = dxs; L.wdg = wdg;
+  L.p1r = p1r; L.am1s = am1s; L.am2s = am2s; L.dxs = dxs; L.wdg = wdg;
   L.xsh = reinterpret_cast<bf16*>(scratch + BW_O_XSH);
   L.p1sh = reinterpret_cast<bf16*>(scratch + BW_O_P1SH);
   L.dY2w = reinterpret_cast<bf16*>(scratch + BW_O_DY2W);
@@ -575,7 +602,7 @@
 constexpr int AUX_BYTES = AUX_CORR + MAX_TRAIN_BATCH * 4;
 static_assert(AUX_BYTES <= MAX_TRAIN_BATCH * F0 * 4, "FC side buffers must fit in dact2");
 
-constexpr int S_O_RAW = 0, S_O_P1R = 3072, S_O_AM1 = S_O_P1R + 2368, S_O_AM2 = S_O_AM1 + 1184,
+constexpr int S_O_P1R = 0, S_O_AM1 = S_O_P1R + 2368, S_O_AM2 = S_O_AM1 + 1184,
               S_O_X = S_O_AM2 + 416, S_O_DX = S_O_X + F0P * 2, S_O_WDG = S_O_DX + F0 * 4,
               S_O_FC = S_O_WDG + 16 * BW_WDGS * 2, S_O_W1C = S_O_FC + 2048, S_O_W2C = S_O_W1C + 16 * 136 * 2,
               S_O_SCR = S_O_W2C + 16 * 232 * 2;
@@ -616,9 +643,9 @@
 }
 
 __global__ __launch_bounds__(NT_CONV) void lenet_sample_step(
-    const uint8_t* __restrict__ images, int sample_base, int nb,
+    const bf16* __restrict__ xprep,
+    int nb,
     const bf16* __restrict__ pk, const float* __restrict__ params,
-    uint32_t seed, const int* __restrict__ round_ctr, int augment,
     const int* __restrict__ labels,
     bf16* __restrict__ act2T,
     bf16* __restrict__ h1T,
@@ -630,10 +657,8 @@
   const int s = blockIdx.x;
   if (s >= nb) return;
   [[maybe_unused]] const int stamp_wg = s;
-  const int gidx = sample_base + s;
   const int tid = threadIdx.x, lane = lane_id(), wave = wave_id();
   const int kq = (lane >> 4) * 8, n16 = lane & 15, rq = (lane >> 4) * 4;
-  uint8_t* raw = smem + S_O_RAW;
   bf16* p1r = reinterpret_cast<bf16*>(smem + S_O_P1R);
   uint8_t* am1s = smem + S_O_AM1;
   uint8_t* am2s = smem + S_O_AM2;
@@ -644,47 +669,47 @@
   float* red = reinterpret_cast<float*>(smem + S_O_RED);
   bf16* xcl = reinterpret_cast<bf16*>(smem + S_O_RED + S_R_XCL);
   bf16* p1cl = reinterpret_cast<bf16*>(smem + S_O_RED + S_R_P1);
-  const BwdLds L = bwd_lds(smem + S_O_SCR, raw, p1r, am1s, am2s, dxs, wdg);
+  const BwdLds L = bwd_lds(smem + S_O_SCR, p1r, am1s, am2s, dxs, wdg);
   FEDMI_STAMP(0, 0);
 
   bf16* w1c = reinterpret_cast<bf16*>(smem + S_O_W1C);
   bf16* w2c = reinterpret_cast<bf16*>(smem + S_O_W2C);
   bf16* w3s = reinterpret_cast<bf16*>(smem + S_O_W3);
   float bias1, bias2;
-  Aug a;
   {
-    constexpr int NI = IMG_BYTES / 16, NWD = 16 * KDGP / 8, NW1 = 16 * K1C / 8, NW2 = 16 * K2C / 8, NW3 = 16 * 96 / 8;
-    constexpr int E1 = NI, E2 = E1 + NWD, E3 = E2 + NW1, E4 = E3 + NW2, E5 = E4 + NW3;
-    static_assert(E5 <= 2 * NT_CONV, "stage: two chunks per thread");
-    uint4 v[2] = {make_uint4(0, 0, 0, 0), make_uint4(0, 0, 0, 0)};
+    constexpr int NWD = 16 * KDGP / 8, NW1 = 16 * K1C / 8, NW2 = 16 * K2C / 8, NW3 = 16 * 96 / 8;
+    constexpr int NCH = 3;
+    constexpr int E1 = XP_CHUNKS, E2 = E1 + NWD, E3 = E2 + NW1, E4 = E3 + NW2, E5 = E4 + NW3;
+    static_assert(E5 <= NCH * NT_CONV, "stage: three chunks per thread");
+    static_assert(XP_ELEMS == 36 * 40 * 4 && (S_O_RED + S_R_XCL) % 16 == 0, "the prepared image is xcl, 16-B chunks");
+    uint4 v[NCH];
 #ifdef FEDMI_STAMPS
     const int dg = fedmi_ks1_diag;
-    const size_t img_sample = (dg & 2) ? 0 : (size_t)gidx;
+    const size_t img_sample = (dg & 2) ? 0 : (size_t)s;
     const int lim = (dg & 1) ? E1 : E5;
 #else
-    const size_t img_sample = (size_t)gidx;
+    const size_t img_sample = (size_t)s;
     constexpr int lim = E5;
 #endif
-#pragma unroll
-    for (int u = 0; u < 2; ++u) {
+    static_assert(PK_W2DG % 8 == 0 && PK_W1C % 8 == 0 && PK_W2C % 8 == 0 && PK_FC3 % 8 == 0, "16-B chunks");
+    const uint4* xp4 = reinterpret_cast<const uint4*>(xprep + img_sample * XP_ELEMS);
+    const uint4* pk4 = reinterpret_cast<const uint4*>(pk);
+#pragma unroll
+    for (int u = 0; u < NCH; ++u) {
       const int e = tid + u * NT_CONV;
-      if (e < E1) v[u] = reinterpret_cast<const uint4*>(images + img_sample * IMG_BYTES)[e];
-      else if (e >= lim) {}
-      else if (e < E2) v[u] = reinterpret_cast<const uint4*>(pk + PK_W2DG)[e - E1];
-      else if (e < E3) v[u] = reinterpret_cast<const uint4*>(pk + PK_W1C)[e - E2];
-      else if (e < E4) v[u] = reinterpret_cast<const uint4*>(pk + PK_W2C)[e - E3];
-      else if (e < E5) v[u] = reinterpret_cast<const uint4*>(pk + PK_FC3)[e - E4];
+      const int wo = e < E2 ? PK_W2DG / 8 + (e - E1) : e < E3 ? PK_W1C / 8 + (e - E2)
+                   : e < E4 ? PK_W2C / 8 + (e - E3) : PK_FC3 / 8 + (e - E4);
+      const uint4* src = (e >= E1 && e < lim) ? pk4 + wo : xp4 + min(e, E1 - 1);
+      v[u] = *src;
     }
     bias1 = n16 < C1 ? params[P_C1B + n16] : 0.f;
     bias2 = params[P_C2B + n16];
-    a = aug_params(augment, seed, round_ctr, gidx);
-    zero_lds<NT_CONV>(xcl, 36 * 40 * 4 * 2);
     bwd_zero(L);
 #pragma unroll
-    for (int u = 0; u < 2; ++u) {
+    for (int u = 0; u < NCH; ++u) {
       const int e = tid + u * NT_CONV;
       if (e < E1) {
-        reinterpret_cast<uint4*>(raw)[e] = v[u];
+        reinterpret_cast<uint4*>(xcl)[e] = v[u];
       } else if (e < E2) {
         const int w = e - E1, row = w / (KDGP / 8), col = w - row * (KDGP / 8);
         reinterpret_cast<uint4*>(wdg + row * BW_WDGS)[col] = v[u];
@@ -707,15 +732,10 @@
   }
   __syncthreads();
   FEDMI_STAMP(1, 7);
+  FEDMI_STAMP(0, 1);
   bf16x8 wb1[4];
 #pragma unroll
   for (int ks = 0; ks < 4; ++ks) wb1[ks] = ld8(w1c + n16 * S_W1C_LD + ks * 32 + kq);
-  for (int e = tid; e < IMG_BYTES; e += NT_CONV) {
-    const int c = e >> 10, y = (e >> 5) & 31, x = e & 31;
-    xcl[(y * 40 + x) * 4 + c] = (bf16)aug_pixel(raw, a, c, y, x);
-  }
-  __syncthreads();
-  FEDMI_STAMP(0, 1);
 
   auto c1_row = [&](int tt) {
     const int q = tt * 4 + (n16 >> 2), y = 2 * (q / P1) + ((n16 >> 1) & 1), x = 2 * (q % P1) + (n16 & 1);
@@ -980,14 +1000,19 @@
 
 constexpr int SGD_NA = (CS + 15) / 16;
 
+FEDMI_DEV float sgd_update(int i, float grad, float p, float m, float* __restrict__ params, float* __restrict__ mom,
+                           float lr, float momentum, float wd) {
+  const float d = __builtin_fmaf(wd, p, grad);
+  const float b = __builtin_fmaf(momentum, m, d);
+  const float np = __builtin_fmaf(-lr, b, p);
+  mom[i] = b;
+  params[i] = np;
+  return np;
+}
+
 FEDMI_DEV void sgd_apply(int i, float grad, float p, float m, float* __restrict__ params, float* __restrict__ mom,
                          bf16* __restrict__ pk, float lr, float momentum, float wd) {
-  const float d = grad + wd * p;
-  const float b = momentum * m + d;
-  const float np = p - lr * b;
-  mom[i] = b;
-  params[i] = np;
-  pack_one(i, np, pk);
+  pack_one(i, sgd_update(i, grad, p, m, params, mom, lr, momentum, wd), pk);
 }
 
 FEDMI_DEV bf16x8 mask_cols(bf16x8 v, int s0, int nb) {
@@ -1036,13 +1061,23 @@
     const float* __restrict__ conv_slab, int nb,
     const bf16* __restrict__ act2T, const bf16* __restrict__ h1T, const unsigned char* __restrict__ aux,
     const bf16* __restrict__ dZ1T, float lr, float momentum, float wd,
-    int* __restrict__ round_ctr, Stats* __restrict__ stats)
+    int* __restrict__ round_ctr, Stats* __restrict__ stats,
+    const uint8_t* __restrict__ images, int next_base, int next_nb, uint32_t seed,
+    const int* __restrict__ aug_ctr, int augment, bf16* __restrict__ xprep)
 {
   __shared__ float red[16][17];
+  __shared__ __attribute__((aligned(16))) uint8_t raw[IMG_BYTES];
   const int b = blockIdx.x, tid = threadIdx.x, wave = wave_id(), lane = lane_id();
   const int n16 = lane & 15, rq = (lane >> 4) * 4;
   [[maybe_unused]] const int stamp_wg = b;
   FEDMI_STAMP(3, 0);
+  if (b >= SGD2_GRID) {
+    const int pb = b - SGD2_GRID, sp = pb / PREP_SPLIT;
+    if (sp < next_nb)
+      prep_sample(images, next_base + sp, pb - sp * PREP_SPLIT, seed, aug_ctr, augment, xprep + (size_t)sp * XP_ELEMS, raw);
+    FEDMI_STAMP(3, 1);
+    return;
+  }
   if (b < SGD_NA) {
     const int pl = tid & 15, g = tid >> 4;
     const int i = b * 16 + pl;
@@ -1078,9 +1113,11 @@
       const f32x4 acc = batch_tile(dZ1T + (size_t)nt * 16 * DZ1_LD, act2T + (size_t)ft * 16 * MAX_TRAIN_BATCH, nb,
                                    params, mom, idx, p, m);
       FEDMI_STAMP(3, 2);
+      bf16* pk1 = pk + PK_FC1 + (nt * 16 + rq) * F0P + ft * 16 + n16;
 #pragma unroll
       for (int r = 0; r < 4; ++r)
-        if (idx[r] >= 0) sgd_apply(idx[r], acc[r], p[r], m[r], params, mom, pk, lr, momentum, wd);
+        if (idx[r] >= 0)
+          pk1[r * F0P] = (bf16)sgd_update(idx[r], acc[r], p[r], m[r], params, mom, lr, momentum, wd);
       FEDMI_STAMP(3, 3);
     }
   } else if (b < SGD_NA + SGD2_NB + SGD2_NC) {
@@ -1097,9 +1134,16 @@
       }
       const f32x4 acc = batch_tile(dz2t + (size_t)nt * 16 * MAX_TRAIN_BATCH, h1T + (size_t)ft * 16 * MAX_TRAIN_BATCH, nb,
                                    params, mom, idx, p, m);
+      const int n0 = nt * 16 + rq, f = ft * 16 + n16;
+      bf16* pk2 = pk + PK_FC2 + n0 * 128 + f;
+      bf16* pk2t = pk + PK_FC2T + f * 96 + n0;
 #pragma unroll
       for (int r = 0; r < 4; ++r)
-        if (idx[r] >= 0) sgd_apply(idx[r], acc[r], p[r], m[r], params, mom, pk, lr, momentum, wd);
+        if (idx[r] >= 0) {
+          const bf16 v = (bf16)sgd_update(idx[r], acc[r], p[r], m[r], params, mom, lr, momentum, wd);
+          pk2[r * 128] = v;
+          pk2t[r] = v;
+        }
     }
   } else if (b < SGD_NA + SGD2_NB + SGD2_NC + SGD2_ND) {
     const int t = (b - SGD_NA - SGD2_NB - SGD2_NC) * 4 + wave;
@@ -1114,9 +1158,11 @@
         idx[r] = (n < NCLS && f < F2) ? P_F3W + n * F2 + f : -1;
       }
       const f32x4 acc = batch_tile(dz3t, h2t + (size_t)t * 16 * MAX_TRAIN_BATCH, nb, params, mom, idx, p, m);
+      bf16* pk3 = pk + PK_FC3 + rq * 96 + t * 16 + n16;
 #pragma unroll
       for (int r = 0; r < 4; ++r)
-        if (idx[r] >= 0) sgd_apply(idx[r], acc[r], p[r], m[r], params, mom, pk, lr, momentum, wd);
+        if (idx[r] >= 0)
+          pk3[r * 96] = (bf16)sgd_update(idx[r], acc[r], p[r], m[r], params, mom, lr, momentum, wd);
     }
   } else {
     const int e = b - (SGD_NA + SGD2_NB + SGD2_NC + SGD2_ND);
@@ -1154,11 +1200,22 @@
     __syncthreads();
     if (e < SGD2_NE && g == 0 && j < 214) {
       const float sum = (bsum[0][tid] + bsum[1][tid]) + (bsum[2][tid] + bsum[3][tid]);
-      sgd_apply(bi, sum, bp, bm, params, mom, pk, lr, momentum, wd);
+      sgd_update(bi, sum, bp, bm, params, mom, lr, momentum, wd);
     }
   }
   if (b == 0 && tid == 0 && round_ctr) atomicAdd(round_ctr, 1);
   FEDMI_STAMP(3, 1);
+}
+
+__global__ __launch_bounds__(PREP_NT) void lenet_prep_batch(
+    const uint8_t* __restrict__ images, int sample_base, int nb, uint32_t seed,
+    const int* __restrict__ round_ctr, int augment, bf16* __restrict__ xprep)
+{
+  __shared__ __attribute__((aligned(16))) uint8_t raw[IMG_BYTES];
+  const int sp = blockIdx.x / PREP_SPLIT;
+  if (sp >= nb) return;
+  prep_sample(images, sample_base + sp, blockIdx.x - sp * PREP_SPLIT, seed, round_ctr, augment,
+              xprep + (size_t)sp * XP_ELEMS, raw);
 }
 
 namespace fedmi {
@@ -1241,20 +1298,34 @@
   hipLaunchKernelGGL(lenet_pack, dim3((P_TOTAL + 255) / 256), dim3(256), 0, st, params, pk);
 }
 
-void launch_lenet_sample_step(hipStream_t st, const uint8_t* images, int sample_base, int nb, const bf16* pk,
-                              const float* params, uint32_t seed, const int* round_ctr, int augment,
+void launch_lenet_prep_batch(hipStream_t st, const uint8_t* images, int sample_base, int nb, uint32_t seed,
+                             const int* round_ctr, int augment, bf16* xprep) {
+  if (nb <= 0 || nb > MAX_TRAIN_BATCH) throw std::invalid_argument("lenet_prep_batch: batch must be in [1, 128]");
+  if (sample_base < 0) throw std::invalid_argument("lenet_prep_batch: negative first sample");
+  hipLaunchKernelGGL(lenet_prep_batch, dim3(nb * PREP_SPLIT), dim3(PREP_NT), 0, st, images, sample_base, nb, seed,
+                     round_ctr, augment, xprep);
+}
+
+void launch_lenet_sample_step(hipStream_t st, const bf16* xprep, int nb, const bf16* pk, const float* params,
                               const int* labels, bf16* act2T, bf16* h1T, float* aux, bf16* dZ1T, float* conv_slab) {
   if (nb <= 0 || nb > MAX_TRAIN_BATCH) throw std::invalid_argument("lenet_sample_step: batch must be in [1, 128]");
-  hipLaunchKernelGGL(lenet_sample_step, dim3(nb), dim3(NT_CONV), 0, st, images, sample_base, nb, pk, params, seed,
-                     round_ctr, augment, labels, act2T, h1T, reinterpret_cast<unsigned char*>(aux), dZ1T, conv_slab);
+  hipLaunchKernelGGL(lenet_sample_step, dim3(nb), dim3(NT_CONV), 0, st, xprep, nb, pk, params, labels, act2T, h1T,
+                     reinterpret_cast<unsigned char*>(aux), dZ1T, conv_slab);
 }
 
 void launch_lenet_sgd2(hipStream_t st, float* params, float* mom, bf16* pk, const float* conv_slab, int nb,
                        const bf16* act2T, const bf16* h1T, const float* aux, const bf16* dZ1T, float lr,
-                       float momentum, float wd, int* round_ctr, Stats* stats) {
+                       float momentum, float wd, int* round_ctr, Stats* stats, const uint8_t* images, int next_base,
+                       int next_nb, uint32_t seed, const int* aug_ctr, int augment, bf16* xprep) {
   if (nb <= 0 || nb > MAX_TRAIN_BATCH) throw std::invalid_argument("lenet_sgd2: batch must be in [1, 128]");
-  hipLaunchKernelGGL(lenet_sgd2, dim3(SGD2_GRID), dim3(256), 0, st, params, mom, pk, conv_slab, nb, act2T, h1T,
-                     reinterpret_cast<const unsigned char*>(aux), dZ1T, lr, momentum, wd, round_ctr, stats);
-}
-
-}
+  if (next_nb < 0 || next_nb > MAX_TRAIN_BATCH || (next_nb > 0 && next_base < 0))
+    throw std::invalid_argument("lenet_sgd2: next batch must be in [0, 128]");
+  if (next_nb > 0 && round_ctr != nullptr)
+    throw std::invalid_argument("lenet_sgd2: the launch that bumps the round counter prepares no batch");
+  static_assert(PREP_NT == 256, "prep blocks are KS2 blocks");
+  hipLaunchKernelGGL(lenet_sgd2, dim3(SGD2_GRID + next_nb * PREP_SPLIT), dim3(256), 0, st, params, mom, pk, conv_slab,
+                     nb, act2T, h1T, reinterpret_cast<const unsigned char*>(aux), dZ1T, lr, momentum, wd, round_ctr,
+                     stats, images, next_base, next_nb, seed, aug_ctr, augment, xprep);
+}
+
+}
diff --git a/csrc/kernels/lenet_layout.h b/csrc/kernels/lenet_layout.h
--- a/csrc/kernels/lenet_layout.h
+++ b/csrc/kernels/lenet_layout.h
@@ -40,6 +40,9 @@
 constexpr int PK_FC3  = PK_FC2T + 128 * 96;
 constexpr int PK_TOTAL = PK_FC3 + 16 * 96;
 
+constexpr int XP_H = 36, XP_W = 40, XP_C = 4;
+constexpr int XP_ELEMS = XP_H * XP_W * XP_C;
+
 constexpr int MAX_TRAIN_BATCH = 128;
 constexpr int FC_SPW = 16;
 constexpr int DZ1_LD = 128;
diff --git a/csrc/runtime/lenet_engine.cpp b/csrc/runtime/lenet_engine.cpp
--- a/csrc/runtime/lenet_engine.cpp
+++ b/csrc/runtime/lenet_engine.cpp
@@ -13,10 +13,12 @@
                           lenet::Stats*);
 void launch_lenet_pack(hipStream_t, const float*, bf16*);
 void launch_lenet_zero_stats(hipStream_t, lenet::Stats*);
-void launch_lenet_sample_step(hipStream_t, const uint8_t*, int, int, const bf16*, const float*, uint32_t, const int*,
-                              int, const int*, bf16*, bf16*, float*, bf16*, float*);
+void launch_lenet_prep_batch(hipStream_t, const uint8_t*, int, int, uint32_t, const int*, int, bf16*);
+void launch_lenet_sample_step(hipStream_t, const bf16*, int, const bf16*, const float*, const int*, bf16*, bf16*,
+                              float*, bf16*, float*);
 void launch_lenet_sgd2(hipStream_t, float*, float*, bf16*, const float*, int, const bf16*, const bf16*, const float*,
-                       const bf16*, float, float, float, int*, lenet::Stats*);
+                       const bf16*, float, float, float, int*, lenet::Stats*, const uint8_t*, int, int, uint32_t,
+                       const int*, int, bf16*);
 
 void check_hip(hipError_t e, const char* what) {
   if (e != hipSuccess) throw std::runtime_error(std::string("fedmi HIP error in ") + what + ": " + hipGetErrorString(e));
@@ -25,7 +27,7 @@
 LeNetEngine::LeNetEngine(const LeNetBuffers& b, SgdConfig sgd, uint32_t seed, bool augment)
     : b_(b), sgd_(sgd), seed_(seed), augment_(augment) {
   if (!b.params || !b.mom || !b.pk || !b.act2 || !b.act2T || !b.h1 || !b.dact2 || !b.dZ1T || !b.conv_slab ||
-      !b.eval_part || !b.train_stats || !b.eval_stats || !b.round_ctr)
+      !b.eval_part || !b.train_stats || !b.eval_stats || !b.round_ctr || !b.xprep)
     throw std::invalid_argument("LeNetEngine: missing device buffer");
   if (b.act2_rows < lenet::MAX_TRAIN_BATCH) throw std::invalid_argument("LeNetEngine: act2_rows < 128");
   check_hip(hipStreamCreateWithFlags(&cap_stream_, hipStreamNonBlocking), "hipStreamCreate");
@@ -59,22 +61,44 @@
   drop_graph();
 }
 
+void LeNetEngine::check_batch(int start, int nb, const char* what) const {
+  if (nb <= 0 || nb > lenet::MAX_TRAIN_BATCH || start < 0 || start + nb > b_.n_train)
+    throw std::invalid_argument(std::string(what) + ": batch out of range");
+}
+
+void LeNetEngine::prep(hipStream_t st, int start, int nb) {
+  check_batch(start, nb, "LeNetEngine::prep");
+  launch_lenet_prep_batch(st, b_.train_images, start, nb, seed_, b_.round_ctr, augment_ ? 1 : 0, b_.xprep);
+  check_hip(hipGetLastError(), "LeNetEngine::prep launch");
+}
+
+void LeNetEngine::launch_step(hipStream_t st, int start, int nb, bool bump_round, int next_start, int next_nb) {
+  check_batch(start, nb, "LeNetEngine::step");
+  if (next_nb != 0) check_batch(next_start, next_nb, "LeNetEngine::step (next batch)");
+  launch_lenet_sample_step(st, b_.xprep, nb, b_.pk, b_.params, b_.train_labels + start, b_.act2T, b_.h1, b_.dact2,
+                           b_.dZ1T, b_.conv_slab);
+  launch_lenet_sgd2(st, b_.params, b_.mom, b_.pk, b_.conv_slab, nb, b_.act2T, b_.h1, b_.dact2, b_.dZ1T, sgd_.lr,
+                    sgd_.momentum, sgd_.weight_decay, bump_round ? b_.round_ctr : nullptr, b_.train_stats,
+                    b_.train_images, next_start, next_nb, seed_, b_.round_ctr, augment_ ? 1 : 0, b_.xprep);
+  check_hip(hipGetLastError(), "LeNetEngine::step launch");
+}
+
 void LeNetEngine::step(hipStream_t st, int start, int nb, bool bump_round, bool reset_stats) {
-  using namespace lenet;
-  if (nb <= 0 || nb > MAX_TRAIN_BATCH || start < 0 || start + nb > b_.n_train)
-    throw std::invalid_argument("LeNetEngine::step: batch out of range");
-  const int aug = augment_ ? 1 : 0;
+  check_batch(start, nb, "LeNetEngine::step");
   if (reset_stats) launch_lenet_zero_stats(st, b_.train_stats);
-  launch_lenet_sample_step(st, b_.train_images, start, nb, b_.pk, b_.params, seed_, b_.round_ctr, aug,
-                           b_.train_labels + start, b_.act2T, b_.h1, b_.dact2, b_.dZ1T, b_.conv_slab);
-  launch_lenet_sgd2(st, b_.params, b_.mom, b_.pk, b_.conv_slab, nb, b_.act2T, b_.h1, b_.dact2, b_.dZ1T, sgd_.lr,
-                    sgd_.momentum, sgd_.weight_decay, bump_round ? b_.round_ctr : nullptr, b_.train_stats);
-  check_hip(hipGetLastError(), "LeNetEngine::step launch");
+  prep(st, start, nb);
+  launch_step(st, start, nb, bump_round, 0, 0);
 }
 
 void LeNetEngine::enqueue_epoch(hipStream_t st) {
   const size_t n = starts_.size();
-  for (size_t i = 0; i < n; ++i) step(st, starts_[i], sizes_[i], i + 1 == n, i == 0);
+  if (n == 0) return;
+  launch_lenet_zero_stats(st, b_.train_stats);
+  prep(st, starts_[0], sizes_[0]);
+  for (size_t i = 0; i < n; ++i) {
+    const bool last = i + 1 == n;
+    launch_step(st, starts_[i], sizes_[i], last, last ? 0 : starts_[i + 1], last ? 0 : sizes_[i + 1]);
+  }
 }
 
 void LeNetEngine::run_epoch(hipStream_t st, bool use_graph) {
diff --git a/csrc/runtime/lenet_engine.h b/csrc/runtime/lenet_engine.h
--- a/csrc/runtime/lenet_engine.h
+++ b/csrc/runtime/lenet_engine.h
@@ -27,6 +27,7 @@
   lenet::Stats* train_stats = nullptr;
   lenet::Stats* eval_stats = nullptr;
   int* round_ctr = nullptr;
+  bf16* xprep = nullptr;
 };
 
 struct SgdConfig {
@@ -52,6 +53,9 @@
 
  private:
   void enqueue_epoch(hipStream_t st);
+  void check_batch(int start, int nb, const char* what) const;
+  void prep(hipStream_t st, int start, int nb);
+  void launch_step(hipStream_t st, int start, int nb, bool bump_round, int next_start, int next_nb);
   void drop_graph();
 
   LeNetBuffers b_;
diff --git a/fedmi/engine/lenet_native.py b/fedmi/engine/lenet_native.py
--- a/fedmi/engine/lenet_native.py
+++ b/fedmi/engine/lenet_native.py
@@ -62,13 +62,14 @@
             self.eval_part = z(2 * ((self.act2_rows + L["FC_SPW"] - 1) // L["FC_SPW"]))
             self.stats = z(2, 4, dt=torch.int32)
             self.round_ctr = z(4, dt=torch.int32)
+            self.xprep = z(B, L["XP_ELEMS"], dt=torch.bfloat16)
         self._bufs = dict(
             train_images=_ptr(self.train_set.x), train_labels=_ptr(self.train_set.y), n_train=len(self.train_set),
             params=_ptr(self.params), mom=_ptr(self.mom), pk=_ptr(self.pk), act2=_ptr(self.act2),
             act2_rows=self.act2_rows, act2T=_ptr(self.act2T), h1=_ptr(self.h1), dact2=_ptr(self.dact2),
             dZ1T=_ptr(self.dZ1T), conv_slab=_ptr(self.conv_slab), eval_part=_ptr(self.eval_part),
             eval_part_floats=self.eval_part.numel(), train_stats=_ptr(self.stats[0]),
-            eval_stats=_ptr(self.stats[1]), round_ctr=_ptr(self.round_ctr))
+            eval_stats=_ptr(self.stats[1]), round_ctr=_ptr(self.round_ctr), xprep=_ptr(self.xprep))
         self.engine = nat.LeNetEngine(self._bufs, cfg.lr, cfg.momentum, cfg.weight_decay, cfg.seed & 0xFFFFFFFF,
                                       bool(data.augment and cfg.augment))
         self._views = ordered_views(self.params, LENET_SPEC)
```

Result: faster. 5.951 million samples/s, median of 6 (+5.0%).
